# lpiccinelli-eth/UniDepth

Hardware: NVIDIA H100
Metric: images/sec UniDepthV2.infer ViT-L/14 480x640 (higher is better)
Workload: dtype f16 operands, f32 accumulate/residual

## Files before the change

include/udb.h:

```cpp
#ifndef UDB_H_
#define UDB_H_
#include <stddef.h>
#include <stdint.h>

#ifdef __cplusplus
extern "C" {
#endif

#define UDB_VERSION 1

int udb_version(void);

typedef struct udb_profile_entry_t {
  char name[48];
  float ms;
  double flops;
  double bytes;
} udb_profile_entry_t;
int udb_profile_begin(void* stream);
int udb_profile_end(udb_profile_entry_t* out, int32_t cap);
const char* udb_last_error(void);
int64_t udb_launch_count(void);

enum { UDB_A_MATRIX = 0, UDB_A_CONV3X3 = 1 };
enum { UDB_ACT_NONE = 0, UDB_ACT_GELU = 1, UDB_ACT_LEAKY = 2 };
enum { UDB_STORE_ROWS = 0, UDB_STORE_CONVT = 1, UDB_STORE_CONVTILE = 2, UDB_STORE_HEAD = 3 };

typedef struct udb_gemm_t {
  const void* a;
  const void* w;
  int32_t M, N, K;
  int32_t lda, ldw;
  int32_t a_mode;
  int32_t conv_B, conv_H, conv_W, conv_C, conv_inH, conv_inW, conv_off, conv_TH, conv_TW;
  int32_t conv_cstride, conv_coff;
  const float* bias;
  const float* gamma;
  const void* resid;
  int32_t resid_f32;
  void* out;
  int32_t out_f32;
  void* out2;
  int32_t out2_leaky;
  int32_t act;
  int32_t store_mode;
  int64_t ldc;
  int32_t rows_per_group, group_stride, row_offset;
  int32_t resid_mod, resid_row_offset;
  int64_t ldr;
  int32_t ct_k, ct_cout, ct_h, ct_w, ct_pad;
  const float* head_w;
  float head_b, head_add;
  int32_t a_split_k;
  int32_t out_split;
  float* ln_stats_out;
  const float* ln_stats_in;
  const float* ln_c1;
  int32_t ln_parts, ln_part_cols;
  float ln_eps;
} udb_gemm_t;

int udb_gemm_f16(const udb_gemm_t* g, void* stream);

typedef struct udb_conv_halo_t {
  const void* x;
  const void* w;
  const float* bias;
  int32_t B, H, W, C, cstride, coff, cout, act;
  void* out;
  int64_t ldc;
  const float* head_w;
  float head_b, head_add;
  float* head_out;
} udb_conv_halo_t;
int udb_conv3x3_halo_f16(const udb_conv_halo_t* c, void* stream);

typedef struct udb_attn_t {
  const void* q;
  const void* k;
  const void* v;
  void* out;
  int32_t B, heads, seq_q, seq_k, head_dim;
  int32_t ldq, ldk, ldv, ldo;
  int32_t q_col0, k_col0, v_col0, o_col0;
  float scale;
  int32_t split;
  int32_t lo_off_q, lo_off_k, lo_off_v, lo_off_o;
} udb_attn_t;

int udb_attention_f16(const udb_attn_t* a, void* stream);

typedef struct udb_layernorm_t {
  const void* in;
  int32_t in_f32;
  void* out;
  int32_t out_f32;
  const float* weight;
  const float* bias;
  int32_t rows, dim;
  int64_t ld_in, ld_out;
  int32_t rows_per_group, group_stride, row_offset;
  float eps;
  int32_t dim_valid;
  int32_t out_split;
} udb_layernorm_t;

int udb_layernorm(const udb_layernorm_t* p, void* stream);

typedef struct udb_preprocess_t {
  const void* rgb;
  int32_t rgb_is_u8;
  int32_t normalize;
  int32_t B, H, W;
  int32_t pad_l, pad_r, pad_t, pad_b;
  int32_t net_h, net_w;
  void* patches;
  int32_t ldp;
  int32_t split;
} udb_preprocess_t;

int udb_preprocess_patchify(const udb_preprocess_t* p, void* stream);

int udb_posembed_bicubic(const float* grid, int32_t m, int32_t dim, float* out, int32_t gh,
                         int32_t gw, void* stream);

int udb_set_cls_rows(float* x, const float* cls_token, const float* pos0, int32_t B, int32_t T,
                     int32_t D, void* stream);
int udb_set_cls_rows_ln(float* x, void* x16, float* stats, const float* cls_token, const float* pos0, int32_t B, int32_t T,
                        int32_t D, int32_t parts, int32_t part_cols, void* stream);

typedef struct udb_small_linear_t {
  const float* x;
  const float* w;
  const float* bias;
  const float* gamma;
  const float* resid;
  float* y;
  int32_t M, N, K;
  int32_t act;
  int32_t ldx, ldy, ldr;
} udb_small_linear_t;
int udb_small_linear_f32(const udb_small_linear_t* p, void* stream);

int udb_camera_attn4_f32(const float* q, const float* kv, const float* pos, float* out, int32_t B,
                         int32_t C, int32_t heads, void* stream);

int udb_camera_intrinsics(const float* x, int32_t B, int32_t net_h, int32_t net_w, float factor,
                          int32_t pad_l, int32_t pad_t, float* intr4, float* k_net, float* k_out,
                          void* stream);

int udb_camera_adjust_k(const float* K, int32_t B, float factor, int32_t pad_l, int32_t pad_t,
                        float* intr4, void* stream);

typedef struct udb_ray_embed_t {
  const float* intr4;
  const float* rays_in;
  const float* scales;
  int32_t B, net_h, net_w, gh, gw, bands;
  void* out;
  int32_t out_f32;
} udb_ray_embed_t;
int udb_ray_embed(const udb_ray_embed_t* p, void* stream);

int udb_upsample2x_nhwc_f16(const void* in, void* out, int32_t B, int32_t H, int32_t W, int32_t C,
                            void* stream);

int udb_resize_ac_pad_nhwc_f16(const void* in, void* out, int32_t B, int32_t H, int32_t W,
                               int32_t C, int32_t oh, int32_t ow, int32_t pad, void* stream);

int udb_reflect_pad1_nhwc_f16(const void* in, void* out, int32_t B, int32_t H, int32_t W, int32_t C,
                              void* stream);

int udb_reflect_border_fill_nhwc_f16(void* buf, int32_t B, int32_t H, int32_t W, int32_t C, void* stream);


typedef struct udb_v1_preprocess_t {
  const void* rgb;
  int32_t rgb_is_u8, scale255, normalize;
  int32_t B, H, W;
  int32_t rh, rw, pad_l, pad_t;
  int32_t net_h, net_w;
  int32_t patch;
  void* patches;
} udb_v1_preprocess_t;
int udb_v1_preprocess(const udb_v1_preprocess_t* p, void* stream);

int udb_vit_tap(const float* x, void* acc, float* cls_out, int32_t B, int32_t N, int32_t D, int32_t first, void* stream);

typedef struct udb_layernorm_any_t {
  const void* in;
  int32_t in_f32;
  void* out;
  int32_t out_f32;
  const float* weight;
  const float* bias;
  int64_t rows;
  int32_t dim;
  int64_t ld_in, ld_out;
  float eps;
  const float* add;
  int64_t add_mod;
  int32_t s2d_h, s2d_w;
} udb_layernorm_any_t;
int udb_layernorm_any(const udb_layernorm_any_t* p, void* stream);

int udb_dwconv7_nhwc_f16(const void* x, const float* w, const float* bias, void* y, int32_t B, int32_t H, int32_t W,
                         int32_t C, void* stream);

int udb_max_accum_f16(const void* src, void* dst, int64_t n, int32_t first, void* stream);

int udb_spatial_mean_f32(const float* x, float* out, int32_t B, int32_t HW, int32_t C, void* stream);

int udb_aa_resize_nhwc_f16(const void* in, void* out, int32_t B, int32_t H, int32_t W, int32_t C, int32_t oh, int32_t ow,
                           void* stream);

typedef struct udb_v1_rays_t {
  const float* intr4;
  int32_t B, net_h, net_w, gh, gw;
  const float* ln_w;
  const float* ln_b;
  void* out;
  float sh_k[81];
} udb_v1_rays_t;
int udb_v1_rays_sh81(const udb_v1_rays_t* p, void* stream);

int udb_v1_camera_intrinsics(const float* x4, const float* gt_k, int32_t B, int32_t net_h, int32_t net_w, float ratio,
                             int32_t pad_l, int32_t pad_t, int32_t skip_camera, float* intr4_rays, float* k_out,
                             float* k4_points, void* stream);

int udb_cross_attn_small(const float* q, const float* q_pos, const void* kv, float* out, float* scratch, int32_t B, int32_t nq,
                         int32_t nk, int32_t D, float scale, void* stream);

int udb_softmax_rows(const float* s, void* p, int64_t rows, int32_t n_valid, int32_t ld_in, int32_t ld_out, float scale,
                     void* stream);

int udb_add_f32(const float* a, const float* b, float* out, void* out_f16, int64_t n, void* stream);

int udb_copy_rows_f32_to_f16(const float* src, void* dst, int32_t groups, int32_t rows_per_group, int32_t D,
                             int64_t dst_group_stride, int64_t dst_row0, void* stream);

int udb_conv3x3_c1_exp(const void* x, const float* w, float bias, float* out, int32_t B, int32_t H, int32_t W, int32_t C,
                       void* stream);

int udb_nystrom_landmarks(const void* q, int32_t ldq, const void* kv, int32_t ldkv, void* out, int32_t B, int32_t n,
                          int32_t heads, void* stream);
int udb_nystrom_k2_pinv(const void* landmarks, float* k2, float* z, float* tmp, int32_t B, int32_t heads, int32_t iters,
                        void* stream);
int udb_nystrom_zk3(const float* z, const void* k3, int32_t ldk3, void* out, int32_t ldo, int32_t B, int32_t heads, void* stream);

int udb_v1_mean_maps(const float* o8, const float* o4, const float* o2, float* mean, int32_t B, int32_t gh, int32_t gw,
                     int32_t net_h, int32_t net_w, void* stream);
typedef struct udb_v1_postprocess_t {
  const float* mean;
  const float* k4;
  int32_t B, net_h, net_w, pad_l, pad_r, pad_t, pad_b, H, W;
  float* out_depth;
  float* out_points;
} udb_v1_postprocess_t;
int udb_v1_postprocess(const udb_v1_postprocess_t* p, void* stream);

typedef struct udb_postprocess_t {
  const float* radius;
  const float* confidence;
  const float* intr4;
  const float* rays_in;
  int32_t B, net_h, net_w, padded_h, padded_w, pad_l, pad_t, H, W;
  float* out_confidence;
  float* out_radius;
  float* out_depth;
  float* out_points;
  float* out_rays;
} udb_postprocess_t;
int udb_postprocess(const udb_postprocess_t* p, void* stream);

typedef struct udb_engine udb_engine;

enum { UDB_DT_F16 = 0, UDB_DT_F32 = 1 };

typedef struct udb_config_t {
  int32_t embed_dim, depth, enc_heads;
  int32_t taps[4];
  int32_t pos_grid;
  int32_t hidden, dec_heads, expansion, out_dim;
  int32_t n_stages;
  int32_t dec_depths[4];
  double ratio_min, ratio_max;
  double pixels_min, pixels_max;
} udb_config_t;

int udb_create(const udb_config_t* cfg, udb_engine** out);
void udb_destroy(udb_engine* e);

int udb_set_weight(udb_engine* e, const char* name, const void* dev_ptr, const int64_t* shape, int32_t ndim,
                   int32_t dtype);
int udb_set_scalar(udb_engine* e, const char* name, double value);

typedef struct udb_geometry_t {
  int32_t pad_l, pad_r, pad_t, pad_b;
  int32_t padded_h, padded_w;
  int32_t net_h, net_w;
  int32_t gh, gw;
  double factor;
} udb_geometry_t;
#define UDB_LEVEL_NETWORK_ONLY (-2)
int udb_geometry(const udb_engine* e, int32_t H, int32_t W, int32_t resolution_level, udb_geometry_t* out);

size_t udb_workspace_bytes(udb_engine* e, int32_t B, int32_t H, int32_t W, int32_t resolution_level);
size_t udb_schedule_bytes(udb_engine* e, int32_t B, int32_t H, int32_t W, int32_t resolution_level);

typedef struct udb_infer_args_t {
  const void* rgb;
  int32_t rgb_is_u8, normalize;
  int32_t B, H, W;
  int32_t resolution_level;
  const float* camera_k;
  const float* camera_rays;
  const float* ray_scales;
  void* workspace;
  size_t workspace_bytes;
  float* confidence;
  float* intrinsics;
  float* radius;
  float* depth;
  float* points;
  float* rays;
  float* depth_features;
} udb_infer_args_t;

int udb_infer_v2(udb_engine* e, const udb_infer_args_t* a, void* stream);

typedef struct udb_engine_v1 udb_engine_v1;

#define UDB_V1_ENCODER_CONVNEXT 0
#define UDB_V1_ENCODER_DINOV2 1

typedef struct udb_v1_config_t {
  int32_t depths[4];
  int32_t dims[4];
  int32_t hidden, heads, expansion;
  int32_t dec_depths[3];
  int32_t encoder;
  int32_t net_h, net_w;
} udb_v1_config_t;

int udb_v1_create(const udb_v1_config_t* cfg, udb_engine_v1** out);
void udb_v1_destroy(udb_engine_v1* e);
int udb_v1_set_weight(udb_engine_v1* e, const char* name, const void* dev_ptr, const int64_t* shape, int32_t ndim,
                      int32_t dtype);
int udb_v1_set_scalar(udb_engine_v1* e, const char* name, double value);
typedef struct udb_v1_geometry_t {
  int32_t resized_h, resized_w;
  int32_t pad_l, pad_r, pad_t, pad_b;
  double ratio;
} udb_v1_geometry_t;
int udb_v1_geometry(int32_t H, int32_t W, int32_t net_h, int32_t net_w, udb_v1_geometry_t* out);
size_t udb_v1_workspace_bytes(udb_engine_v1* e, int32_t B, int32_t H, int32_t W);

typedef struct udb_infer_v1_args_t {
  const void* rgb;
  int32_t rgb_is_u8;
  int32_t scale255;
  int32_t normalize;
  int32_t B, H, W;
  const float* intrinsics;
  int32_t skip_camera;
  void* workspace;
  size_t workspace_bytes;
  float* out_intrinsics;
  float* out_points;
  float* out_depth;
} udb_infer_v1_args_t;

int udb_infer_v1(udb_engine_v1* e, const udb_infer_v1_args_t* a, void* stream);

int udb_p2p_alloc(size_t bytes, void** dev_ptr, void* handle64);
int udb_p2p_open(const void* handle64, void** peer_ptr);
int udb_p2p_close(void* peer_ptr);
int udb_p2p_free(void* dev_ptr);
int udb_p2p_barrier(void* const* peer_flags_dev, void* my_flags, int32_t rank, int32_t world, uint32_t epoch,
                    int32_t* timeout_flag_dev, void* stream);
int udb_p2p_copy(void* dst, const void* src, size_t bytes, void* stream);

#ifdef __cplusplus
}
#endif
#endif
```

unidepth_b200/_cabi.py:

```python
from __future__ import annotations

import ctypes as C
import os

_HERE = os.path.dirname(os.path.abspath(__file__))
LIB_PATH = os.environ.get("UDB_LIB", os.path.join(_HERE, "libudb.so"))

A_MATRIX, A_CONV3X3 = 0, 1
ACT_NONE, ACT_GELU, ACT_LEAKY = 0, 1, 2
STORE_ROWS, STORE_CONVT, STORE_CONVTILE, STORE_HEAD = 0, 1, 2, 3

vp, i32, i64, f32 = C.c_void_p, C.c_int32, C.c_int64, C.c_float


class Gemm(C.Structure):
    _fields_ = [
        ("a", vp), ("w", vp), ("M", i32), ("N", i32), ("K", i32), ("lda", i32), ("ldw", i32),
        ("a_mode", i32),
        ("conv_B", i32), ("conv_H", i32), ("conv_W", i32), ("conv_C", i32), ("conv_inH", i32),
        ("conv_inW", i32), ("conv_off", i32), ("conv_TH", i32), ("conv_TW", i32),
        ("conv_cstride", i32), ("conv_coff", i32),
        ("bias", vp), ("gamma", vp), ("resid", vp), ("resid_f32", i32), ("out", vp), ("out_f32", i32),
        ("out2", vp), ("out2_leaky", i32), ("act", i32), ("store_mode", i32), ("ldc", i64),
        ("rows_per_group", i32), ("group_stride", i32), ("row_offset", i32),
        ("resid_mod", i32), ("resid_row_offset", i32), ("ldr", i64),
        ("ct_k", i32), ("ct_cout", i32), ("ct_h", i32), ("ct_w", i32), ("ct_pad", i32),
        ("head_w", vp), ("head_b", f32), ("head_add", f32),
        ("a_split_k", i32), ("out_split", i32),
        ("ln_stats_out", vp), ("ln_stats_in", vp), ("ln_c1", vp), ("ln_parts", i32), ("ln_part_cols", i32), ("ln_eps", f32),
    ]


class ConvHalo(C.Structure):
    _fields_ = [
        ("x", vp), ("w", vp), ("bias", vp),
        ("B", i32), ("H", i32), ("W", i32), ("C", i32), ("cstride", i32), ("coff", i32), ("cout", i32), ("act", i32),
        ("out", vp), ("ldc", i64), ("head_w", vp), ("head_b", f32), ("head_add", f32), ("head_out", vp),
    ]


class Attn(C.Structure):
    _fields_ = [
        ("q", vp), ("k", vp), ("v", vp), ("out", vp),
        ("B", i32), ("heads", i32), ("seq_q", i32), ("seq_k", i32), ("head_dim", i32),
        ("ldq", i32), ("ldk", i32), ("ldv", i32), ("ldo", i32),
        ("q_col0", i32), ("k_col0", i32), ("v_col0", i32), ("o_col0", i32), ("scale", f32),
        ("split", i32), ("lo_off_q", i32), ("lo_off_k", i32), ("lo_off_v", i32), ("lo_off_o", i32),
    ]


class LayerNorm(C.Structure):
    _fields_ = [
        ("inp", vp), ("in_f32", i32), ("out", vp), ("out_f32", i32), ("weight", vp), ("bias", vp),
        ("rows", i32), ("dim", i32), ("ld_in", i64), ("ld_out", i64),
        ("rows_per_group", i32), ("group_stride", i32), ("row_offset", i32), ("eps", f32), ("dim_valid", i32),
        ("out_split", i32),
    ]


class Preprocess(C.Structure):
    _fields_ = [
        ("rgb", vp), ("rgb_is_u8", i32), ("normalize", i32), ("B", i32), ("H", i32), ("W", i32),
        ("pad_l", i32), ("pad_r", i32), ("pad_t", i32), ("pad_b", i32), ("net_h", i32), ("net_w", i32),
        ("patches", vp), ("ldp", i32), ("split", i32),
    ]


class SmallLinear(C.Structure):
    _fields_ = [
        ("x", vp), ("w", vp), ("bias", vp), ("gamma", vp), ("resid", vp), ("y", vp),
        ("M", i32), ("N", i32), ("K", i32), ("act", i32), ("ldx", i32), ("ldy", i32), ("ldr", i32),
    ]


class RayEmbed(C.Structure):
    _fields_ = [
        ("intr4", vp), ("rays_in", vp), ("scales", vp),
        ("B", i32), ("net_h", i32), ("net_w", i32), ("gh", i32), ("gw", i32), ("bands", i32),
        ("out", vp), ("out_f32", i32),
    ]


class Postprocess(C.Structure):
    _fields_ = [
        ("radius", vp), ("confidence", vp), ("intr4", vp), ("rays_in", vp),
        ("B", i32), ("net_h", i32), ("net_w", i32), ("padded_h", i32), ("padded_w", i32),
        ("pad_l", i32), ("pad_t", i32), ("H", i32), ("W", i32),
        ("out_confidence", vp), ("out_radius", vp), ("out_depth", vp), ("out_points", vp), ("out_rays", vp),
    ]


class Config(C.Structure):
    _fields_ = [
        ("embed_dim", i32), ("depth", i32), ("enc_heads", i32), ("taps", i32 * 4), ("pos_grid", i32),
        ("hidden", i32), ("dec_heads", i32), ("expansion", i32), ("out_dim", i32), ("n_stages", i32),
        ("dec_depths", i32 * 4),
        ("ratio_min", C.c_double), ("ratio_max", C.c_double), ("pixels_min", C.c_double), ("pixels_max", C.c_double),
    ]


class Geometry(C.Structure):
    _fields_ = [
        ("pad_l", i32), ("pad_r", i32), ("pad_t", i32), ("pad_b", i32), ("padded_h", i32), ("padded_w", i32),
        ("net_h", i32), ("net_w", i32), ("gh", i32), ("gw", i32), ("factor", C.c_double),
    ]


class V1Geometry(C.Structure):
    _fields_ = [
        ("resized_h", i32), ("resized_w", i32), ("pad_l", i32), ("pad_r", i32), ("pad_t", i32), ("pad_b", i32),
        ("ratio", C.c_double),
    ]


class InferArgs(C.Structure):
    _fields_ = [
        ("rgb", vp), ("rgb_is_u8", i32), ("normalize", i32), ("B", i32), ("H", i32), ("W", i32),
        ("resolution_level", i32), ("camera_k", vp), ("camera_rays", vp), ("ray_scales", vp), ("workspace", vp),
        ("workspace_bytes", C.c_size_t),
        ("confidence", vp), ("intrinsics", vp), ("radius", vp), ("depth", vp), ("points", vp), ("rays", vp),
        ("depth_features", vp),
    ]


class V1Preprocess(C.Structure):
    _fields_ = [
        ("rgb", vp), ("rgb_is_u8", i32), ("scale255", i32), ("normalize", i32), ("B", i32), ("H", i32), ("W", i32),
        ("rh", i32), ("rw", i32), ("pad_l", i32), ("pad_t", i32), ("net_h", i32), ("net_w", i32), ("patch", i32),
        ("patches", vp),
    ]


class LayerNormAny(C.Structure):
    _fields_ = [
        ("inp", vp), ("in_f32", i32), ("out", vp), ("out_f32", i32), ("weight", vp), ("bias", vp),
        ("rows", i64), ("dim", i32), ("ld_in", i64), ("ld_out", i64), ("eps", f32), ("add", vp), ("add_mod", i64),
        ("s2d_h", i32), ("s2d_w", i32),
    ]


class V1Rays(C.Structure):
    _fields_ = [
        ("intr4", vp), ("B", i32), ("net_h", i32), ("net_w", i32), ("gh", i32), ("gw", i32),
        ("ln_w", vp), ("ln_b", vp), ("out", vp), ("sh_k", f32 * 81),
    ]


class V1Postprocess(C.Structure):
    _fields_ = [
        ("mean", vp), ("k4", vp), ("B", i32), ("net_h", i32), ("net_w", i32), ("pad_l", i32), ("pad_r", i32),
        ("pad_t", i32), ("pad_b", i32), ("H", i32), ("W", i32), ("out_depth", vp), ("out_points", vp),
    ]


class V1Config(C.Structure):
    _fields_ = [
        ("depths", i32 * 4), ("dims", i32 * 4), ("hidden", i32), ("heads", i32), ("expansion", i32),
        ("dec_depths", i32 * 3), ("encoder", i32), ("net_h", i32), ("net_w", i32),
    ]


class InferV1Args(C.Structure):
    _fields_ = [
        ("rgb", vp), ("rgb_is_u8", i32), ("scale255", i32), ("normalize", i32), ("B", i32), ("H", i32), ("W", i32),
        ("intrinsics", vp), ("skip_camera", i32), ("workspace", vp), ("workspace_bytes", C.c_size_t),
        ("out_intrinsics", vp), ("out_points", vp), ("out_depth", vp),
    ]


class ProfileEntry(C.Structure):
    _fields_ = [("name", C.c_char * 48), ("ms", f32), ("flops", C.c_double), ("bytes", C.c_double)]


DT_F16, DT_F32 = 0, 1

EXPORTS = {
    "udb_version": (i32, []),
    "udb_last_error": (C.c_char_p, []),
    "udb_launch_count": (i64, []),
    "udb_profile_begin": (i32, [vp]),
    "udb_profile_end": (i32, [C.POINTER(ProfileEntry), i32]),
    "udb_gemm_f16": (i32, [C.POINTER(Gemm), vp]),
    "udb_conv3x3_halo_f16": (i32, [C.POINTER(ConvHalo), vp]),
    "udb_attention_f16": (i32, [C.POINTER(Attn), vp]),
    "udb_layernorm": (i32, [C.POINTER(LayerNorm), vp]),
    "udb_preprocess_patchify": (i32, [C.POINTER(Preprocess), vp]),
    "udb_posembed_bicubic": (i32, [vp, i32, i32, vp, i32, i32, vp]),
    "udb_set_cls_rows": (i32, [vp, vp, vp, i32, i32, i32, vp]),
    "udb_set_cls_rows_ln": (i32, [vp, vp, vp, vp, vp, i32, i32, i32, i32, i32, vp]),
    "udb_small_linear_f32": (i32, [C.POINTER(SmallLinear), vp]),
    "udb_camera_attn4_f32": (i32, [vp, vp, vp, vp, i32, i32, i32, vp]),
    "udb_camera_intrinsics": (i32, [vp, i32, i32, i32, f32, i32, i32, vp, vp, vp, vp]),
    "udb_ray_embed": (i32, [C.POINTER(RayEmbed), vp]),
    "udb_upsample2x_nhwc_f16": (i32, [vp, vp, i32, i32, i32, i32, vp]),
    "udb_resize_ac_pad_nhwc_f16": (i32, [vp, vp, i32, i32, i32, i32, i32, i32, i32, vp]),
    "udb_reflect_pad1_nhwc_f16": (i32, [vp, vp, i32, i32, i32, i32, vp]),
    "udb_reflect_border_fill_nhwc_f16": (i32, [vp, i32, i32, i32, i32, vp]),
    "udb_postprocess": (i32, [C.POINTER(Postprocess), vp]),
    "udb_camera_adjust_k": (i32, [vp, i32, f32, i32, i32, vp, vp]),
    "udb_create": (i32, [C.POINTER(Config), C.POINTER(vp)]),
    "udb_destroy": (None, [vp]),
    "udb_set_weight": (i32, [vp, C.c_char_p, vp, C.POINTER(i64), i32, i32]),
    "udb_set_scalar": (i32, [vp, C.c_char_p, C.c_double]),
    "udb_geometry": (i32, [vp, i32, i32, i32, C.POINTER(Geometry)]),
    "udb_workspace_bytes": (C.c_size_t, [vp, i32, i32, i32, i32]),
    "udb_schedule_bytes": (C.c_size_t, [vp, i32, i32, i32, i32]),
    "udb_infer_v2": (i32, [vp, C.POINTER(InferArgs), vp]),
    "udb_v1_preprocess": (i32, [C.POINTER(V1Preprocess), vp]),
    "udb_layernorm_any": (i32, [C.POINTER(LayerNormAny), vp]),
    "udb_dwconv7_nhwc_f16": (i32, [vp, vp, vp, vp, i32, i32, i32, i32, vp]),
    "udb_max_accum_f16": (i32, [vp, vp, i64, i32, vp]),
    "udb_spatial_mean_f32": (i32, [vp, vp, i32, i32, i32, vp]),
    "udb_vit_tap": (i32, [vp, vp, vp, i32, i32, i32, i32, vp]),
    "udb_aa_resize_nhwc_f16": (i32, [vp, vp, i32, i32, i32, i32, i32, i32, vp]),
    "udb_v1_rays_sh81": (i32, [C.POINTER(V1Rays), vp]),
    "udb_v1_camera_intrinsics": (i32, [vp, vp, i32, i32, i32, f32, i32, i32, i32, vp, vp, vp, vp]),
    "udb_cross_attn_small": (i32, [vp, vp, vp, vp, vp, i32, i32, i32, i32, f32, vp]),
    "udb_softmax_rows": (i32, [vp, vp, i64, i32, i32, i32, f32, vp]),
    "udb_add_f32": (i32, [vp, vp, vp, vp, i64, vp]),
    "udb_copy_rows_f32_to_f16": (i32, [vp, vp, i32, i32, i32, i64, i64, vp]),
    "udb_conv3x3_c1_exp": (i32, [vp, vp, f32, vp, i32, i32, i32, i32, vp]),
    "udb_nystrom_landmarks": (i32, [vp, i32, vp, i32, vp, i32, i32, i32, vp]),
    "udb_nystrom_k2_pinv": (i32, [vp, vp, vp, vp, i32, i32, i32, vp]),
    "udb_nystrom_zk3": (i32, [vp, vp, i32, vp, i32, i32, i32, vp]),
    "udb_v1_mean_maps": (i32, [vp, vp, vp, vp, i32, i32, i32, i32, i32, vp]),
    "udb_v1_postprocess": (i32, [C.POINTER(V1Postprocess), vp]),
    "udb_v1_create": (i32, [C.POINTER(V1Config), C.POINTER(vp)]),
    "udb_v1_destroy": (None, [vp]),
    "udb_v1_set_weight": (i32, [vp, C.c_char_p, vp, C.POINTER(i64), i32, i32]),
    "udb_v1_set_scalar": (i32, [vp, C.c_char_p, C.c_double]),
    "udb_v1_geometry": (i32, [i32, i32, i32, i32, C.POINTER(V1Geometry)]),
    "udb_v1_workspace_bytes": (C.c_size_t, [vp, i32, i32, i32]),
    "udb_infer_v1": (i32, [vp, C.POINTER(InferV1Args), vp]),
    "udb_p2p_alloc": (i32, [C.c_size_t, C.POINTER(vp), vp]),
    "udb_p2p_open": (i32, [vp, C.POINTER(vp)]),
    "udb_p2p_close": (i32, [vp]),
    "udb_p2p_free": (i32, [vp]),
    "udb_p2p_barrier": (i32, [vp, vp, i32, i32, C.c_uint32, vp, vp]),
    "udb_p2p_copy": (i32, [vp, vp, C.c_size_t, vp]),
}

_lib = None


def lib():
    global _lib
    if _lib is None:
        if not os.path.exists(LIB_PATH):
            raise RuntimeError(
                f"{LIB_PATH} not found: build the CUDA extension first (python -m unidepth_b200.build). "
                "unidepth_b200 has no CPU / PyTorch fallback.")
        l = C.CDLL(LIB_PATH)
        for name, (res, args) in EXPORTS.items():
            if "UDB_LIB" in os.environ and not hasattr(l, name):
                continue
            fn = getattr(l, name)
            fn.restype = res
            fn.argtypes = args
        _lib = l
    return _lib


def check(rc: int, what: str):
    if rc != 0:
        raise RuntimeError(f"{what} failed: {lib().udb_last_error().decode()}")


def profile(fn, stream_ptr, cap: int = 4096):
    l = lib()
    check(l.udb_profile_begin(stream_ptr), "udb_profile_begin")
    try:
        fn()
    finally:
        buf = (ProfileEntry * cap)()
        n = l.udb_profile_end(buf, cap)
    if n < 0:
        raise RuntimeError(f"udb_profile_end failed: {l.udb_last_error().decode()}")
    return [(buf[i].name.decode(), buf[i].ms, buf[i].flops, buf[i].bytes) for i in range(min(n, cap))]


def launch_count() -> int:
    return int(lib().udb_launch_count())
```

unidepth_b200/csrc/engine.cu:

```cuda
#include "engine_common.h"

namespace udb {

struct ShapeTables {
  float* pos = nullptr;
  float* scales = nullptr;
};

constexpr int PATCH = 14;

}

struct udb_engine : udb::EngineBase {
  udb_config_t cfg;
  std::unordered_map<long long, udb::ShapeTables> tables;
  std::unordered_map<std::string, size_t> ws_need;
};

namespace udb {

static inline int floordiv2(int v) { return v >= 0 ? v / 2 : -((-v + 1) / 2); }

static void paddings(int H, int W, double lo, double hi, udb_geometry_t* g) {
  const double ratio = static_cast<double>(W) / H;
  const double target = fmin(hi, fmax(lo, ratio));
  g->pad_l = g->pad_r = g->pad_t = g->pad_b = 0;
  if (ratio > target) {
    const int h_new = static_cast<int>(W / target);
    g->pad_t = floordiv2(h_new - H);
    g->pad_b = h_new - H - g->pad_t;
    g->padded_h = h_new;
    g->padded_w = W;
  } else {
    const int w_new = static_cast<int>(H * target);
    g->pad_l = floordiv2(w_new - W);
    g->pad_r = w_new - W - g->pad_l;
    g->padded_h = H;
    g->padded_w = w_new;
  }
}

static int resize(const udb_config_t& c, int level, udb_geometry_t* g) {
  double lo = c.pixels_min, hi = c.pixels_max;
  if (level >= 0) {
    if (level >= 10) { set_error("resolution_level should be in [0, 10)"); return 1; }
    const double interval = (hi - lo) / 10;
    const double l2 = level * interval + lo, h2 = (level + 1) * interval + lo;
    lo = l2;
    hi = h2;
  }
  const double n_ori = static_cast<double>(g->padded_w) * g->padded_h;
  const double target = fmin(hi, fmax(lo, n_ori));
  g->factor = pow(target / n_ori, 0.5);
  const int new_w = static_cast<int>(g->padded_w * g->factor);
  const int new_h = static_cast<int>(g->padded_h * g->factor);
  g->net_h = static_cast<int>(ceil(static_cast<double>(new_h) / PATCH)) * PATCH;
  g->net_w = static_cast<int>(ceil(static_cast<double>(new_w) / PATCH)) * PATCH;
  g->gh = g->net_h / PATCH;
  g->gw = g->net_w / PATCH;
  return 0;
}

static int run(udb_engine* e, const udb_infer_args_t& a, const udb_geometry_t& g, const ShapeTables& tb, Arena& ar,
               void* st) {
  const udb_config_t& cf = e->cfg;
  Ctx c{e, &ar, st, ar.dry};
  const int B = a.B, nh = g.net_h, nw = g.net_w, gh = g.gh, gw = g.gw;
  const int N = gh * gw, T = N + 1, D = cf.embed_dim, hid = cf.hidden;
  const size_t BN = static_cast<size_t>(B) * N, BT = static_cast<size_t>(B) * T;

  Stage stage;
  stage.next("udb:preprocess+patch_embed");
  const bool sp = e->scalars.count("precision") && e->scalars["precision"] == 1.0;
  const int sx = sp ? 2 : 1;
  const bool fuse = !sp && e->scalars.count("fuse_ln") && e->scalars["fuse_ln"] == 1.0;
  const int ln_bn = D % 256 == 0 ? 256 : (D % 192 == 0 ? 192 : (D % 128 == 0 ? 128 : 64));
  const int ln_parts = D / ln_bn * 2, ln_pc = ln_bn / 2;
  __half* x16 = fuse ? ar.h(BT * D) : nullptr;
  float* stats = fuse ? ar.f(BT * ln_parts * 2) : nullptr;
  __half* patches = ar.h(BN * 640 * sx);
  if (!c.dry) {
    udb_preprocess_t p;
    memset(&p, 0, sizeof(p));
    p.rgb = a.rgb; p.rgb_is_u8 = a.rgb_is_u8; p.normalize = a.normalize; p.B = B; p.H = a.H; p.W = a.W;
    p.pad_l = g.pad_l; p.pad_r = g.pad_r; p.pad_t = g.pad_t; p.pad_b = g.pad_b; p.net_h = nh; p.net_w = nw;
    p.patches = patches; p.ldp = 640 * sx; p.split = sp ? 1 : 0;
    c.done(udb_preprocess_patchify(&p, st));
  }
  float* x = ar.f(BT * D);
  {
    Ctx::G q{patches, c.H("patch_w"), static_cast<int>(BN), D, sp ? 3 * 640 : 640};
    q.lda = 640 * sx; q.a_split_k = sp ? 640 : 0;
    q.bias = c.F("patch_b"); q.resid = tb.pos; q.resid_f32 = 1; q.ldr = D; q.out = x; q.out_f32 = 1;
    q.rows_per_group = N; q.group_stride = T; q.row_offset = 1; q.resid_mod = N; q.resid_row_offset = 1;
    c.expect2("patch_w", D, sp ? 3 * 640 : 640);
    if (fuse) { q.out2 = x16; q.out2_leaky = 0; q.ln_stats_out = stats; q.ln_parts = ln_parts; q.ln_part_cols = ln_pc; }
    c.gemm(q);
    if (!c.dry && !c.rc)
      c.done(fuse ? udb_set_cls_rows_ln(x, x16, stats, c.F("cls"), tb.pos, B, T, D, ln_parts, ln_pc, st)
                  : udb_set_cls_rows(x, c.F("cls"), tb.pos, B, T, D, st));
  }

  stage.next("udb:encoder_blocks");
  __half* feats[4];
  float* clss[4];
  for (int l = 0; l < 4; ++l) { feats[l] = ar.h(BN * D); clss[l] = ar.f(static_cast<size_t>(B) * D); }
  {
    VitBlocks v{B, T, D, cf.enc_heads, cf.depth};
    v.split = sp; v.fuse = fuse; v.x16 = x16; v.stats = stats; v.ln_parts = ln_parts; v.ln_pc = ln_pc;
    int tap = 0;
    vit_blocks(c, "blocks.", x, v, [&](int i) {
      if (tap < 4 && i + 1 == cf.taps[tap]) {
        c.layernorm(x, 1, feats[tap], 0, c.F("norm_w"), c.F("norm_b"), static_cast<int>(BN), D, 1e-5f, N, T, 1);
        c.layernorm(x, 1, clss[tap], 1, c.F("norm_w"), c.F("norm_b"), B, D, 1e-5f, 1, T, 0);
        ++tap;
      }
    });
    if (tap != 4 && !c.rc) { set_error("engine: taps must be 4 increasing block indices <= depth"); c.rc = 1; }
  }

  stage.next("udb:adapters+camera_head");
  float* Fl[4];
  for (int l = 0; l < 4; ++l) {
    Fl[l] = ar.f(BN * hid);
    Ctx::G q{feats[l], c.H(idx("adapt.%d.w", l)), static_cast<int>(BN), hid, D};
    q.bias = c.F(idx("adapt.%d.b", l)); q.out = Fl[l]; q.out_f32 = 1;
    c.gemm(q);
  }
  float* tokens = ar.f(static_cast<size_t>(B) * 4 * hid);
  for (int l = 0; l < 4; ++l)
    c.small_linear(clss[l], B, D, c.F(idx("cam_adapt.%d.w", l)), hid, c.F(idx("cam_adapt.%d.b", l)), UDB_ACT_NONE, nullptr,
                   nullptr, tokens + l * hid, D, 4 * hid, 0);

  const int R4 = B * 4;
  float* t = cam_mlp(c, "cam.project", tokens, R4, hid, hid, hid, nullptr, nullptr);
  for (int k = 1; k <= 2; ++k) {
    const std::string ag = idx("cam.agg%d", k);
    float* xn = ar.f(static_cast<size_t>(R4) * hid);
    float* cn = ar.f(static_cast<size_t>(R4) * hid);
    c.layernorm(t, 1, xn, 1, c.F(ag + ".nxw"), c.F(ag + ".nxb"), R4, hid, 1e-5f);
    c.layernorm(t, 1, cn, 1, c.F(ag + ".ncw"), c.F(ag + ".ncb"), R4, hid, 1e-5f);
    float* q = ar.f(static_cast<size_t>(R4) * hid);
    float* kv = ar.f(static_cast<size_t>(R4) * 2 * hid);
    c.small_linear(xn, R4, hid, c.F(ag + ".q"), hid, nullptr, UDB_ACT_NONE, nullptr, nullptr, q);
    c.small_linear(cn, R4, hid, c.F(ag + ".kv"), 2 * hid, nullptr, UDB_ACT_NONE, nullptr, nullptr, kv);
    float* a4 = ar.f(static_cast<size_t>(R4) * hid);
    if (!c.dry && !c.rc) c.done(udb_camera_attn4_f32(q, kv, c.F("cam.pos"), a4, B, hid, cf.dec_heads, st));
    float* t2 = ar.f(static_cast<size_t>(R4) * hid);
    c.small_linear(a4, R4, hid, c.F(ag + ".out"), hid, nullptr, UDB_ACT_NONE, c.F(ag + ".ls1"), t, t2);
    t = cam_mlp(c, ag + ".mlp", t2, R4, hid, cf.expansion * hid, hid, t2, c.F(ag + ".ls2"));
  }
  float* x4 = cam_mlp(c, "cam.pinhole", t, R4, hid, hid, 1, nullptr, nullptr);
  float* intr4 = ar.f(static_cast<size_t>(B) * 4);
  float* k_net = ar.f(static_cast<size_t>(B) * 9);
  if (!c.dry && !c.rc)
    c.done(udb_camera_intrinsics(x4, B, nh, nw, static_cast<float>(g.factor), g.pad_l, g.pad_t, intr4, k_net, a.intrinsics, st));

  stage.next("udb:ray_embedding+prompt_blocks");
  const float* ray_intr = intr4;
  if (a.camera_k && !a.camera_rays) {
    float* gt4 = ar.f(static_cast<size_t>(B) * 4);
    if (!c.dry && !c.rc) c.done(udb_camera_adjust_k(a.camera_k, B, static_cast<float>(g.factor), g.pad_l, g.pad_t, gt4, st));
    ray_intr = gt4;
  }
  float* remb = ar.f(BN * hid);
  if (!c.dry && !c.rc) {
    udb_ray_embed_t p;
    memset(&p, 0, sizeof(p));
    p.intr4 = ray_intr; p.rays_in = a.camera_rays; p.scales = a.ray_scales ? a.ray_scales : tb.scales;
    p.B = B; p.net_h = nh; p.net_w = nw; p.gh = gh; p.gw = gw; p.bands = hid / 2; p.out = remb; p.out_f32 = 1;
    c.done(udb_ray_embed(&p, st));
  }

  __half* cond[4];
  for (int l = 0; l < 4; ++l) cond[l] = ar.h(BN * hid);
  const int hd = hid / cf.dec_heads;
  const int hp = cf.dec_heads * 64;
  {
    const size_t m = ar.mark();
    __half* xn = ar.h(BN * hid);
    __half* cn = ar.h(BN * hid);
    __half* qb = ar.h(BN * hp);
    __half* kvb = ar.h(BN * 2 * hp);
    __half* ab = ar.h(BN * hp);
    __half* mb = ar.h(BN * cf.expansion * hid);
    const float scale = static_cast<float>(pow(static_cast<double>(hd), -0.5));
    for (int l = 0; l < 4; ++l) {
      const std::string p = idx("prompt.%d.", l);
      c.layernorm(Fl[l], 1, xn, 0, c.F(p + "nxw"), c.F(p + "nxb"), static_cast<int>(BN), hid, 1e-5f);
      c.layernorm(remb, 1, cn, 0, c.F(p + "ncw"), c.F(p + "ncb"), static_cast<int>(BN), hid, 1e-5f);
      { Ctx::G q{xn, c.H(p + "q"), static_cast<int>(BN), hp, hid}; q.out = qb; c.gemm(q); }
      { Ctx::G q{cn, c.H(p + "kv"), static_cast<int>(BN), 2 * hp, hid}; q.out = kvb; c.gemm(q); }
      c.attention(qb, kvb, kvb, ab, B, cf.dec_heads, N, N, hp, 2 * hp, 2 * hp, hp, 0, 0, hp, scale);
      { Ctx::G q{ab, c.H(p + "out"), static_cast<int>(BN), hid, hp}; q.resid = Fl[l]; q.resid_f32 = 1; q.out = Fl[l];
        q.out_f32 = 1; c.gemm(q); }
      c.layernorm(Fl[l], 1, xn, 0, c.F(p + "mnw"), c.F(p + "mnb"), static_cast<int>(BN), hid, 1e-5f);
      { Ctx::G q{xn, c.H(p + "w1"), static_cast<int>(BN), cf.expansion * hid, hid}; q.bias = c.F(p + "b1");
        q.act = UDB_ACT_GELU; q.out = mb; c.gemm(q); }
      { Ctx::G q{mb, c.H(p + "w2"), static_cast<int>(BN), hid, cf.expansion * hid}; q.bias = c.F(p + "b2");
        q.resid = Fl[l]; q.resid_f32 = 1; q.out = cond[l]; c.gemm(q); }
    }
    ar.release(m);
  }

  stage.next("udb:upsampling_stages");
  { Ctx::G q{cond[0], c.H("lat_w"), static_cast<int>(BN), hid, hid}; q.bias = c.F("lat_b"); q.out = a.depth_features;
    q.out_f32 = 1; c.gemm(q); }
  const void* prev = a.depth_features;
  int prev_f32 = 1;
  int cur_h = gh, cur_w = gw, c_hr = 0;
  for (int i = 0; i < cf.n_stages; ++i) {
    const std::string s = idx("ups.%d.", i);
    const int k = i == 0 ? 1 : 2 * i;
    const Weight* ctw = c.W(s + "ct_w");
    const int cout = static_cast<int>(ctw->shape[0]) / (k * k);
    const int oh = cur_h, ow = cur_w;
    const size_t px = static_cast<size_t>(B) * oh * ow;
    __half* nxt = nullptr;
    const int up_c = static_cast<int>(c.W(s + "up_w")->shape[0]);
    nxt = ar.h(px * 4 * up_c);
    const size_t m = ar.mark();
    float* lat = ar.f(px * cout);
    __half* act = ar.h(px * cout);
    __half* tmp = ar.h(px * cout);
    c.conv_transpose(cond[i + 1], static_cast<int>(BN), hid, ctw->p, k, cout, gh, gw, c.F(s + "ct_b"), prev, prev_f32, lat, 1,
                     act, 1, 0);
    for (int j = 0; j < cf.dec_depths[i]; ++j) {
      const std::string r = idx2("ups.%d.rcu.%d.", i, j);
      c.expect2(r + "w1", cout, 9 * cout);
      c.expect2(r + "w2", cout, 9 * cout);
      c.conv3x3(act, B, oh, ow, cout, c.H(r + "w1"), cout, c.F(r + "b1"), UDB_ACT_LEAKY, nullptr, nullptr, 0, tmp, 0,
                nullptr, 1);
      c.conv3x3(tmp, B, oh, ow, cout, c.H(r + "w2"), cout, c.F(r + "b2"), UDB_ACT_NONE, c.F(r + "gamma"), lat, 1, lat, 1,
                act, j + 1 < cf.dec_depths[i] ? 1 : 0);
    }
    __half* u = ar.h(px * up_c);
    { Ctx::G q{act, c.H(s + "up_w"), static_cast<int>(px), up_c, cout}; q.bias = c.F(s + "up_b"); q.out = u; c.gemm(q); }
    if (!c.dry && !c.rc) c.done(udb_upsample2x_nhwc_f16(u, nxt, B, oh, ow, up_c, st));
    ar.release(m);
    prev = nxt;
    prev_f32 = 0;
    cur_h = 2 * oh;
    cur_w = 2 * ow;
    c_hr = up_c;
  }
  const int hh = cur_h, hw = cur_w;
  const size_t hpx = static_cast<size_t>(B) * hh * hw;

  stage.next("udb:depth+confidence_heads");
  __half* xhat = ar.h(hpx * c_hr);
  const int nxt_last = (2 * hid) >> cf.n_stages;
  const int c_valid = nxt_last > cf.out_dim ? nxt_last : cf.out_dim;
  c.layernorm(prev, 0, xhat, 0, c.F("ln_ones"), c.F("ln_zeros"), static_cast<int>(hpx), c_hr, 1e-5f, 0, 0, 0,
              c_valid != c_hr ? c_valid : 0);
  const int n_mlp = static_cast<int>(c.W("head_mlp_w")->shape[0]);
  __half* mp = ar.h(static_cast<size_t>(B) * (hh + 2) * (hw + 2) * n_mlp);
  c.conv_transpose(xhat, static_cast<int>(hpx), c_hr, c.H("head_mlp_w"), 1, n_mlp, hh, hw, c.F("head_mlp_b"), nullptr, 0, mp,
                   0, nullptr, 1, 1);
  if (!c.dry && !c.rc) c.done(udb_reflect_border_fill_nhwc_f16(mp, B, hh, hw, n_mlp, st));
  float* planes[2];
  for (int i = 0; i < 2; ++i) {
    const std::string hn = idx("heads.%d.", i);
    const int lr_c = static_cast<int>(c.W(hn + "lr_w")->shape[0]);
    planes[i] = ar.f(static_cast<size_t>(B) * nh * nw);
    const size_t m = ar.mark();
    __half* lr = ar.h(hpx * lr_c);
    c.conv_halo(mp, B, hh, hw, n_mlp / 2, n_mlp, i * (n_mlp / 2), c.H(hn + "lr_w"), lr_c, c.F(hn + "lr_b"), UDB_ACT_NONE, lr,
                nullptr, 0.f, 0.f, nullptr);
    __half* up = ar.h(static_cast<size_t>(B) * (nh + 2) * (nw + 2) * lr_c);
    if (!c.dry && !c.rc) c.done(udb_resize_ac_pad_nhwc_f16(lr, up, B, hh, hw, lr_c, nh, nw, 1, st));
    c.conv_halo(up, B, nh, nw, lr_c, lr_c, 0, c.H(hn + "hr_w"), 32, c.F(hn + "hr_b"), UDB_ACT_LEAKY, nullptr,
                c.F(hn + "head_w"), static_cast<float>(c.S(hn + "head_b")), static_cast<float>(c.S(hn + "add")), planes[i]);
    ar.release(m);
  }

  stage.next("udb:postprocess");
  if (!c.dry && !c.rc) {
    udb_postprocess_t p;
    memset(&p, 0, sizeof(p));
    p.radius = planes[0]; p.confidence = planes[1]; p.intr4 = ray_intr; p.rays_in = a.camera_rays;
    p.B = B; p.net_h = nh; p.net_w = nw; p.padded_h = g.padded_h; p.padded_w = g.padded_w; p.pad_l = g.pad_l; p.pad_t = g.pad_t;
    p.H = a.H; p.W = a.W;
    p.out_confidence = a.confidence; p.out_radius = a.radius; p.out_depth = a.depth; p.out_points = a.points; p.out_rays = a.rays;
    c.done(udb_postprocess(&p, st));
  }
  if (!c.rc && ar.overflow) { set_error("engine: workspace too small (%zu bytes needed)", ar.peak); return 1; }
  return c.rc;
}

static void ray_scale_table(int gh, int gw, int bands, std::vector<float>& out) {
  const int mx = (gh > gw ? gh : gw) / 2;
  const float end = static_cast<float>(log2(static_cast<double>(mx)));
  const float step = bands > 1 ? end / static_cast<float>(bands - 1) : 0.f;
  out.resize(bands);
  for (int i = 0; i < bands; ++i) {
    const float v = i < bands / 2 ? step * i : end - step * (bands - 1 - i);
    out[i] = powf(2.0f, v);
  }
}

static const ShapeTables* prepare(udb_engine* e, const udb_geometry_t& g) {
  const long long key = (static_cast<long long>(g.gh) << 32) | static_cast<unsigned>(g.gw);
  auto it = e->tables.find(key);
  if (it != e->tables.end()) return &it->second;
  auto pw = e->w.find("pos");
  if (pw == e->w.end()) { set_error("engine: 'pos' must be registered before udb_workspace_bytes"); return nullptr; }
  const int D = e->cfg.embed_dim, m = e->cfg.pos_grid, N = g.gh * g.gw;
  ShapeTables tb;
  auto fail = [&tb](const char* why) -> const ShapeTables* {
    if (why) set_error("%s", why);
    cudaFree(tb.pos);
    cudaFree(tb.scales);
    return nullptr;
  };
  if (cudaMalloc(&tb.pos, static_cast<size_t>(N + 1) * D * 4) != cudaSuccess ||
      cudaMalloc(&tb.scales, static_cast<size_t>(e->cfg.hidden / 2) * 4) != cudaSuccess)
    return fail("engine: cudaMalloc of the per-shape tables failed");
  const float* pos = static_cast<const float*>(pw->second.p);
  cudaMemcpy(tb.pos, pos, static_cast<size_t>(D) * 4, cudaMemcpyDeviceToDevice);
  if (g.gh == m && g.gw == m) {
    cudaMemcpy(tb.pos + D, pos + D, static_cast<size_t>(N) * D * 4, cudaMemcpyDeviceToDevice);
  } else if (udb_posembed_bicubic(pos + D, m, D, tb.pos + D, g.gh, g.gw, nullptr)) {
    return fail(nullptr);
  }
  std::vector<float> sc;
  ray_scale_table(g.gh, g.gw, e->cfg.hidden / 2, sc);
  cudaMemcpy(tb.scales, sc.data(), sc.size() * 4, cudaMemcpyHostToDevice);
  if (cudaDeviceSynchronize() != cudaSuccess) return fail("engine: preparing the per-shape tables failed");
  return &(e->tables[key] = tb);
}

}

using namespace udb;

extern "C" {

int udb_create(const udb_config_t* cfg, udb_engine** out) {
  if (!cfg || !out) { set_error("udb_create: null argument"); return 1; }
  if (cfg->embed_dim <= 0 || cfg->embed_dim % 64 || cfg->embed_dim / cfg->enc_heads != 64) {
    set_error("udb_create: encoder needs 64-wide heads (embed_dim %d, heads %d)", cfg->embed_dim, cfg->enc_heads);
    return 1;
  }
  const int hd = cfg->dec_heads > 0 ? cfg->hidden / cfg->dec_heads : 0;
  if (hd <= 0 || hd > 64) { set_error("udb_create: decoder head dim %d not supported", hd); return 1; }
  if (cfg->n_stages < 1 || cfg->n_stages > 4) { set_error("udb_create: n_stages %d out of range", cfg->n_stages); return 1; }
  udb_engine* e = new udb_engine();
  e->cfg = *cfg;
  *out = e;
  return 0;
}

void udb_destroy(udb_engine* e) {
  if (!e) return;
  for (auto& kv : e->tables) {
    cudaFree(kv.second.pos);
    cudaFree(kv.second.scales);
  }
  delete e;
}

int udb_set_weight(udb_engine* e, const char* name, const void* dev_ptr, const int64_t* shape, int32_t ndim, int32_t dtype) {
  if (!e || !name || !dev_ptr || ndim < 0 || ndim > 4) { set_error("udb_set_weight: bad argument"); return 1; }
  if (reinterpret_cast<uintptr_t>(dev_ptr) & 15) { set_error("udb_set_weight(%s): pointer must be 16-byte aligned", name); return 1; }
  Weight w;
  w.p = dev_ptr;
  w.dtype = dtype;
  w.ndim = ndim;
  for (int i = 0; i < ndim; ++i) w.shape[i] = shape[i];
  e->w[name] = w;
  return 0;
}

int udb_set_scalar(udb_engine* e, const char* name, double value) {
  if (!e || !name) { set_error("udb_set_scalar: bad argument"); return 1; }
  e->scalars[name] = value;
  return 0;
}

int udb_geometry(const udb_engine* e, int32_t H, int32_t W, int32_t level, udb_geometry_t* out) {
  if (!e || !out || H <= 0 || W <= 0) { set_error("udb_geometry: bad argument"); return 1; }
  if (level == UDB_LEVEL_NETWORK_ONLY) {
    if (H % PATCH || W % PATCH) { set_error("network-only input %dx%d must be a multiple of %d", H, W, PATCH); return 1; }
    memset(out, 0, sizeof(*out));
    out->padded_h = out->net_h = H;
    out->padded_w = out->net_w = W;
    out->gh = H / PATCH;
    out->gw = W / PATCH;
    out->factor = 1.0;
    return 0;
  }
  paddings(H, W, e->cfg.ratio_min, e->cfg.ratio_max, out);
  return resize(e->cfg, level, out);
}

size_t udb_schedule_bytes(udb_engine* e, int32_t B, int32_t H, int32_t W, int32_t level) {
  if (!e || B <= 0) { set_error("udb_schedule_bytes: bad argument"); return 0; }
  udb_geometry_t g;
  if (udb_geometry(e, H, W, level, &g)) return 0;
  udb_infer_args_t a;
  memset(&a, 0, sizeof(a));
  a.B = B; a.H = H; a.W = W; a.resolution_level = level;
  a.camera_k = reinterpret_cast<const float*>(16);
  const ShapeTables none;
  Arena ar(nullptr, 0);
  if (run(e, a, g, none, ar, nullptr)) return 0;
  return ar.peak + 256;
}

size_t udb_workspace_bytes(udb_engine* e, int32_t B, int32_t H, int32_t W, int32_t level) {
  udb_geometry_t g;
  if (udb_geometry(e, H, W, level, &g)) return 0;
  const ShapeTables* tb = prepare(e, g);
  if (!tb) return 0;
  udb_infer_args_t a;
  memset(&a, 0, sizeof(a));
  a.B = B; a.H = H; a.W = W; a.resolution_level = level;
  a.camera_k = reinterpret_cast<const float*>(16);
  Arena ar(nullptr, 0);
  if (run(e, a, g, *tb, ar, nullptr)) return 0;
  char key[96];
  snprintf(key, sizeof(key), "%d,%d,%d,%d", B, H, W, level);
  e->ws_need[key] = ar.peak + 256;
  return ar.peak + 256;
}

int udb_infer_v2(udb_engine* e, const udb_infer_args_t* a, void* stream) {
  if (!e || !a || !a->rgb || !a->workspace) { set_error("udb_infer_v2: null argument"); return 1; }
  if (!a->confidence || !a->intrinsics || !a->radius || !a->depth || !a->points || !a->rays || !a->depth_features) {
    set_error("udb_infer_v2: all seven output pointers are required");
    return 1;
  }
  udb_geometry_t g;
  if (udb_geometry(e, a->H, a->W, a->resolution_level, &g)) return 1;
  const long long key = (static_cast<long long>(g.gh) << 32) | static_cast<unsigned>(g.gw);
  auto it = e->tables.find(key);
  char wkey[96];
  snprintf(wkey, sizeof(wkey), "%d,%d,%d,%d", a->B, a->H, a->W, a->resolution_level);
  auto need = e->ws_need.find(wkey);
  if (it == e->tables.end() || need == e->ws_need.end()) {
    set_error("udb_infer_v2: shape %dx%dx%d (level %d) not prepared; call udb_workspace_bytes first", a->B, a->H, a->W,
              a->resolution_level);
    return 1;
  }
  if (a->workspace_bytes < need->second) {
    set_error("udb_infer_v2: workspace too small (%zu bytes given, %zu needed)", a->workspace_bytes, need->second);
    return 1;
  }
  Arena ar(a->workspace, a->workspace_bytes);
  if (reinterpret_cast<uintptr_t>(a->workspace) & 255) { set_error("udb_infer_v2: workspace must be 256-byte aligned"); return 1; }
  return run(e, *a, g, it->second, ar, stream);
}

}
```

unidepth_b200/csrc/gemm.cu:

```cuda
#include "common.h"
#include "ptx.cuh"

namespace udb {

constexpr int BM = 128;
constexpr int BK = 64;
constexpr int kEpiWarps = 8;
constexpr int kTP = 36;
constexpr int kThreads = (kEpiWarps + 4) * 32;

struct GemmArgs {
  int M, N, K, num_kb;
  int tiles_m, tiles_n;
  int a_mode;
  int conv_B, conv_H, conv_W, conv_cpb , conv_off, conv_TH, conv_TW, conv_tx, conv_ty;
  const float* bias;
  const float* gamma;
  const void* resid;
  int resid_f32;
  void* out;
  int out_f32;
  __half* out2;
  int out2_leaky;
  int act;
  int store_mode;
  long long ldc, ldr;
  int rpg, gstride, roff;
  int resid_mod, resid_roff;
  int ct_k, ct_cout, ct_h, ct_w, ct_pad;
  int conv_coff;
  const float* head_w;
  float head_b, head_add;
  int a_wrap;
  int out_split;
  float* stats_out;
  const float* ln_stats;
  const float* ln_c1;
  int ln_parts, ln_part_cols;
  float ln_eps;
};

template <int BN>
struct GemmCfg {
  static constexpr int kStages = BN >= 256 ? 3 : (BN >= 192 ? 4 : (BN >= 128 ? 5 : 7));
  static constexpr int kABytes = BM * BK * 2;
  static constexpr int kBBytes = BN * BK * 2;
  static constexpr int kStageBytes = kABytes + kBBytes;
  static constexpr int kStagingBytes = kEpiWarps * (32 * kTP * 4 + 2 * 32 * 4);
  static constexpr int kSmemBytes = kStages * kStageBytes + kStagingBytes + 256 ;
  static_assert(kSmemBytes <= 232448, "shared memory per block");
};

struct EpiWarp {
  float* T;
  float* Twg;
  uint32_t* roff_out;
  uint32_t* roff_res;
  int wg, wq, grp, lane, r_in_tile;
};

template <int BN, bool LNF>
__device__ __forceinline__ void epilogue_tile(const GemmArgs& p, const EpiWarp& w, const float (&acc)[BN / 2], const int mt,
                                              const int nt) {
  constexpr int kGroups = BN >= 64 ? 2 : 1;
  constexpr int kColsPerGrp = BN / kGroups;
  const int grp = w.grp, lane = w.lane, r_in_tile = w.r_in_tile;
  const bool active = grp < kGroups;
  float* T = w.T;
  uint32_t* roff_out = w.roff_out;
  uint32_t* roff_res = w.roff_res;
  bool valid = false;
  long long out_off = 0, res_off = 0;
  uint32_t vmask = 0;
  float ln_mean = 0.f, ln_rstd = 1.f;
  float st_pivot = 0.f, st_s1 = 0.f, st_s2 = 0.f;
  bool st_first = true;
  if (active) {

    const int m = mt * BM + r_in_tile;
    if (p.store_mode == UDB_STORE_CONVTILE || p.store_mode == UDB_STORE_HEAD) {
      const int per_img = p.conv_tx * p.conv_ty;
      const int b = mt / per_img;
      const int r = mt % per_img;
      const int y = (r / p.conv_tx) * p.conv_TH + r_in_tile / p.conv_TW;
      const int x = (r % p.conv_tx) * p.conv_TW + r_in_tile % p.conv_TW;
      valid = (b < p.conv_B) && (y < p.conv_H) && (x < p.conv_W);
      out_off = (((long long)b * p.conv_H + y) * p.conv_W + x) * p.ldc;
      res_off = (((long long)b * p.conv_H + y) * p.conv_W + x) * p.ldr;
    } else if (p.store_mode == UDB_STORE_CONVT) {
      valid = m < p.M;
      const int hw = p.ct_h * p.ct_w;
      const int b = m / hw;
      const int r = m % hw;
      const int y = r / p.ct_w, x = r % p.ct_w;
      const long long W2 = (long long)p.ct_w * p.ct_k + 2 * p.ct_pad;
      const long long H2 = (long long)p.ct_h * p.ct_k + 2 * p.ct_pad;
      out_off = ((b * H2 + (long long)y * p.ct_k + p.ct_pad) * W2 + (long long)x * p.ct_k + p.ct_pad) * p.ct_cout;
      res_off = out_off;
    } else {
      valid = m < p.M;
      long long orow = m;
      if (p.rpg > 0) orow = (long long)(m / p.rpg) * p.gstride + (m % p.rpg) + p.roff;
      out_off = orow * p.ldc;
      res_off = (p.resid_mod > 0) ? ((long long)(m % p.resid_mod) + p.resid_roff) * p.ldr
                                  : orow * p.ldr;
    }
    vmask = __ballot_sync(0xffffffffu, valid);
    roff_out[lane] = static_cast<uint32_t>(out_off);
    roff_res[lane] = static_cast<uint32_t>(res_off);
    __syncwarp();
    if (LNF && p.ln_stats) {
      const float2* sp = reinterpret_cast<const float2*>(p.ln_stats) + (long long)(valid ? m : 0) * p.ln_parts;
      float ms = 0.f, m2 = 0.f;
      for (int q = 0; q < p.ln_parts; ++q) ms += sp[q].x;
      ln_mean = ms / (float)p.ln_parts;
      for (int q = 0; q < p.ln_parts; ++q) {
        const float2 t = sp[q];
        m2 += t.y + (float)p.ln_part_cols * (t.x - ln_mean) * (t.x - ln_mean);
      }
      ln_rstd = rsqrtf(m2 / (float)(p.ln_parts * p.ln_part_cols) + p.ln_eps);
    }
  }
  const int frow = 16 * (w.wq & 1) + (lane >> 2), fcol = 2 * (lane & 3);
#pragma unroll
  for (int c = 0; c < kColsPerGrp; c += 32) {
    bar_sync(1 + w.wg, 128);
#pragma unroll
    for (int gi = 0; gi < kGroups; ++gi) {
      float* Tt = w.Twg + ((w.wq >> 1) | (gi << 1)) * 32 * kTP;
#pragma unroll
      for (int j = 0; j < 4; ++j) {
        const int f = ((gi * kColsPerGrp + c) / 8 + j) * 4;
        *reinterpret_cast<float2*>(Tt + frow * kTP + 8 * j + fcol) = make_float2(acc[f], acc[f + 1]);
        *reinterpret_cast<float2*>(Tt + (frow + 8) * kTP + 8 * j + fcol) = make_float2(acc[f + 2], acc[f + 3]);
      }
    }
    bar_sync(1 + w.wg, 128);
    if (!active) continue;
    const int col = grp * kColsPerGrp + c;
    const int n0 = nt * BN + col;
    float v[32];
#pragma unroll
    for (int j = 0; j < 32; j += 4) {
      const float4 t = *reinterpret_cast<const float4*>(T + lane * kTP + j);
      v[j] = t.x; v[j + 1] = t.y; v[j + 2] = t.z; v[j + 3] = t.w;
    }
    __syncwarp();
    if (n0 >= p.N) continue;
    if (LNF && p.ln_stats) {
      const float4* cp = reinterpret_cast<const float4*>(p.ln_c1 + n0);
      const float mr = ln_mean * ln_rstd;
#pragma unroll
      for (int j = 0; j < 8; ++j) {
        const float4 c4 = __ldg(cp + j);
        v[4 * j] = fmaf(v[4 * j], ln_rstd, -mr * c4.x);
        v[4 * j + 1] = fmaf(v[4 * j + 1], ln_rstd, -mr * c4.y);
        v[4 * j + 2] = fmaf(v[4 * j + 2], ln_rstd, -mr * c4.z);
        v[4 * j + 3] = fmaf(v[4 * j + 3], ln_rstd, -mr * c4.w);
      }
    }
    if (p.bias) {
      const float4* bp = reinterpret_cast<const float4*>(p.bias + n0);
#pragma unroll
      for (int j = 0; j < 8; ++j) {
        const float4 b4 = __ldg(bp + j);
        v[4 * j] += b4.x; v[4 * j + 1] += b4.y; v[4 * j + 2] += b4.z; v[4 * j + 3] += b4.w;
      }
    }
    if (p.act == UDB_ACT_GELU) {
#pragma unroll
      for (int j = 0; j < 32; j += 2) gelu_erf_pair(v[j], v[j + 1]);
    } else if (p.act == UDB_ACT_LEAKY) {
#pragma unroll
      for (int j = 0; j < 32; ++j) v[j] = leaky(v[j]);
    }
    if (p.store_mode == UDB_STORE_HEAD) {
      float head = p.head_b;
#pragma unroll
      for (int j = 0; j < 32; ++j) head = fmaf(v[j], __ldg(p.head_w + j), head);
      head = fminf(fmaxf(head, -8.0f), 8.0f) + p.head_add;
      if (valid) reinterpret_cast<float*>(p.out)[out_off] = expf(head);
      continue;
    }
    if (p.gamma) {
      const float4* gp = reinterpret_cast<const float4*>(p.gamma + n0);
#pragma unroll
      for (int j = 0; j < 8; ++j) {
        const float4 g4 = __ldg(gp + j);
        v[4 * j] *= g4.x; v[4 * j + 1] *= g4.y; v[4 * j + 2] *= g4.z; v[4 * j + 3] *= g4.w;
      }
    }
    long long coff = n0;
    if (p.store_mode == UDB_STORE_CONVT) {
      const int tap = n0 / p.ct_cout;
      const int co = n0 % p.ct_cout;
      const long long W2 = (long long)p.ct_w * p.ct_k + 2 * p.ct_pad;
      coff = ((long long)(tap / p.ct_k) * W2 + (tap % p.ct_k)) * p.ct_cout + co;
    }
    const uint32_t c32 = static_cast<uint32_t>(coff);
    const int l4 = (lane & 7) * 4, rq = lane >> 3;
    float* Trow = T + lane * kTP;
    auto stage_rows = [&](const float (&x)[32]) {
#pragma unroll
      for (int j = 0; j < 32; j += 4)
        *reinterpret_cast<float4*>(Trow + j) = make_float4(x[j], x[j + 1], x[j + 2], x[j + 3]);
    };
    auto for_rows = [&](auto&& body) {
      if (vmask == 0xffffffffu) {
#pragma unroll
        for (int i = 0; i < 8; ++i) body(4 * i + rq, true);
      } else {
#pragma unroll
        for (int i = 0; i < 8; ++i) body(4 * i + rq, ((vmask >> (4 * i + rq)) & 1u) != 0);
      }
    };
    if (p.resid) {
      if (p.resid_f32) {
        const float* rp = reinterpret_cast<const float*>(p.resid) + c32 + l4;
        float4 tmp[8];
        int k = 0;
        for_rows([&](int rr, bool ok) {
          tmp[k++] = ok ? *reinterpret_cast<const float4*>(rp + roff_res[rr]) : make_float4(0.f, 0.f, 0.f, 0.f);
        });
#pragma unroll
        for (int i = 0; i < 8; ++i) *reinterpret_cast<float4*>(T + (4 * i + rq) * kTP + l4) = tmp[i];
      } else {
        const __half* rp = reinterpret_cast<const __half*>(p.resid) + c32 + l4;
        uint2 tmp[8];
        int k = 0;
        for_rows([&](int rr, bool ok) {
          tmp[k++] = ok ? *reinterpret_cast<const uint2*>(rp + roff_res[rr]) : make_uint2(0u, 0u);
        });
#pragma unroll
        for (int i = 0; i < 8; ++i) {
          const float2 a = __half22float2(*reinterpret_cast<const __half2*>(&tmp[i].x));
          const float2 b = __half22float2(*reinterpret_cast<const __half2*>(&tmp[i].y));
          *reinterpret_cast<float4*>(T + (4 * i + rq) * kTP + l4) = make_float4(a.x, a.y, b.x, b.y);
        }
      }
      __syncwarp();
#pragma unroll
      for (int j = 0; j < 32; j += 4) {
        const float4 t = *reinterpret_cast<const float4*>(Trow + j);
        v[j] += t.x; v[j + 1] += t.y; v[j + 2] += t.z; v[j + 3] += t.w;
      }
      __syncwarp();
    }
    if (LNF && p.stats_out) {
      if (st_first) { st_pivot = v[0]; st_first = false; }
#pragma unroll
      for (int j = 0; j < 32; ++j) {
        const float dlt = v[j] - st_pivot;
        st_s1 += dlt;
        st_s2 = fmaf(dlt, dlt, st_s2);
      }
    }
    if (p.out) {
      stage_rows(v);
      __syncwarp();
      if (p.out_f32) {
        float* op = reinterpret_cast<float*>(p.out) + c32 + l4;
        for_rows([&](int rr, bool ok) {
          if (ok) *reinterpret_cast<float4*>(op + roff_out[rr]) = *reinterpret_cast<const float4*>(T + rr * kTP + l4);
        });
      } else {
        __half* op = reinterpret_cast<__half*>(p.out) + c32 + l4;
        if (p.out_split == 0) {
          for_rows([&](int rr, bool ok) {
            const float4 t = *reinterpret_cast<const float4*>(T + rr * kTP + l4);
            if (ok) *reinterpret_cast<uint2*>(op + roff_out[rr]) = make_uint2(pack_half2(t.x, t.y), pack_half2(t.z, t.w));
          });
        } else {
          for_rows([&](int rr, bool ok) {
            const float4 t = *reinterpret_cast<const float4*>(T + rr * kTP + l4);
            const uint2 hi = make_uint2(pack_half2(t.x, t.y), pack_half2(t.z, t.w));
            const float2 h01 = __half22float2(*reinterpret_cast<const __half2*>(&hi.x));
            const float2 h23 = __half22float2(*reinterpret_cast<const __half2*>(&hi.y));
            if (ok) {
              *reinterpret_cast<uint2*>(op + roff_out[rr]) = hi;
              *reinterpret_cast<uint2*>(op + roff_out[rr] + p.out_split) =
                  make_uint2(pack_half2(t.x - h01.x, t.y - h01.y), pack_half2(t.z - h23.x, t.w - h23.y));
            }
          });
        }
      }
      __syncwarp();
    }
    if (p.out2) {
      if (p.out2_leaky) {
#pragma unroll
        for (int j = 0; j < 32; ++j) v[j] = leaky(v[j]);
        stage_rows(v);
      } else if (!p.out) {
        stage_rows(v);
      }
      __syncwarp();
      __half* op = p.out2 + c32 + l4;
      for_rows([&](int rr, bool ok) {
        const float4 t = *reinterpret_cast<const float4*>(T + rr * kTP + l4);
        if (ok) *reinterpret_cast<uint2*>(op + roff_out[rr]) = make_uint2(pack_half2(t.x, t.y), pack_half2(t.z, t.w));
      });
      __syncwarp();
    }
  }
  if (LNF && p.stats_out && active && valid && !st_first) {
    const float n = (float)kColsPerGrp;
    const float mean_p = st_pivot + st_s1 / n;
    const float m2_p = fmaxf(st_s2 - st_s1 * st_s1 / n, 0.f);
    const long long orow = out_off / p.ldc;
    reinterpret_cast<float2*>(p.stats_out)[orow * (p.tiles_n * kGroups) + nt * kGroups + grp] = make_float2(mean_p, m2_p);
  }
}

template <int BN, bool LNF>
__global__ void __launch_bounds__(kThreads, 1)
gemm_f16_kernel(const __grid_constant__ CUtensorMap tmA, const __grid_constant__ CUtensorMap tmB,
                const GemmArgs p) {
  using Cfg = GemmCfg<BN>;
  constexpr int kStages = Cfg::kStages;
  extern __shared__ __align__(1024) uint8_t smem[];
  uint8_t* sA = smem;
  uint8_t* sB = smem + kStages * Cfg::kABytes;
  uint8_t* staging = smem + kStages * Cfg::kStageBytes;
  uint64_t* bars = reinterpret_cast<uint64_t*>(staging + Cfg::kStagingBytes);
  uint64_t* full_bar = bars;
  uint64_t* empty_bar = bars + kStages;

  const int warp = threadIdx.x >> 5;
  const int lane = threadIdx.x & 31;
  pdl_launch_dependents();

  if (threadIdx.x == 0) {
    if (smem_u32(smem) & 1023) __trap();
    prefetch_tmap(&tmA);
    prefetch_tmap(&tmB);
    for (int i = 0; i < kStages; ++i) {
      mbar_init(&full_bar[i], 1);
      mbar_init(&empty_bar[i], kEpiWarps);
    }
    fence_barrier_init();
  }
  __syncthreads();
  pdl_wait();

  const int num_tiles = p.tiles_m * p.tiles_n;

  if (warp >= kEpiWarps) {
    setmaxnreg_dec<40>();
    if (warp != kEpiWarps) return;
    const bool elected = elect_one();
    int stage = 0;
    uint32_t phase = 0;
    for (int tile = blockIdx.x; tile < num_tiles; tile += gridDim.x) {
      const int mt = tile / p.tiles_n;
      const int nt = tile % p.tiles_n;
      int cb = 0, cy = 0, cx = 0;
      if (p.a_mode == UDB_A_CONV3X3) {
        const int per_img = p.conv_tx * p.conv_ty;
        cb = mt / per_img;
        const int r = mt % per_img;
        cy = (r / p.conv_tx) * p.conv_TH + p.conv_off;
        cx = (r % p.conv_tx) * p.conv_TW + p.conv_off;
      }
      for (int kb = 0; kb < p.num_kb; ++kb) {
        mbar_wait(&empty_bar[stage], phase ^ 1);
        if (elected) {
          mbar_arrive_expect_tx(&full_bar[stage], Cfg::kStageBytes);
          if (p.a_mode == UDB_A_CONV3X3) {
            const int tap = kb / p.conv_cpb;
            const int c0 = p.conv_coff + (kb % p.conv_cpb) * BK;
            tma_load_4d(sA + stage * Cfg::kABytes, &tmA, &full_bar[stage], c0, cx + tap % 3, cy + tap / 3, cb);
          } else {
            int ka = kb * BK;
            if (p.a_wrap && ka >= p.a_wrap) ka -= p.a_wrap;
            tma_load_2d(sA + stage * Cfg::kABytes, &tmA, &full_bar[stage], ka, mt * BM);
          }
          tma_load_2d(sB + stage * Cfg::kBBytes, &tmB, &full_bar[stage], kb * BK, nt * BN);
        }
        __syncwarp();
        if (++stage == kStages) {
          stage = 0;
          phase ^= 1;
        }
      }
    }
  } else {
    setmaxnreg_inc<232>();
    const int wg = warp >> 2, wq = warp & 3;
    float* Twg = reinterpret_cast<float*>(staging) + wg * 4 * 32 * kTP;
    uint32_t* roff = reinterpret_cast<uint32_t*>(staging + kEpiWarps * 32 * kTP * 4) + warp * 64;
    const EpiWarp ctx{Twg + wq * 32 * kTP, Twg, roff, roff + 32, wg, wq, wq >> 1, lane, 64 * wg + 32 * (wq & 1) + lane};
    float acc[BN / 2];
#pragma unroll
    for (int i = 0; i < BN / 2; ++i) acc[i] = 0.f;
    int stage = 0;
    uint32_t phase = 0;
    for (int tile = blockIdx.x; tile < num_tiles; tile += gridDim.x) {
      const int mt = tile / p.tiles_n;
      const int nt = tile % p.tiles_n;
      int prev = -1;
      for (int kb = 0; kb < p.num_kb; ++kb) {
        mbar_wait(&full_bar[stage], phase);
        const uint64_t da = gmma_desc_sw128(smem_u32(sA + stage * Cfg::kABytes + wg * 64 * 128), 16, 1024);
        const uint64_t db = gmma_desc_sw128(smem_u32(sB + stage * Cfg::kBBytes), 16, 1024);
        wgmma_fence();
#pragma unroll
        for (int k = 0; k < BK / 16; ++k) WgmmaSS<BN>::run(acc, da + 2 * k, db + 2 * k, (kb | k) != 0 ? 1u : 0u);
        wgmma_commit();
        wgmma_wait<1>();
        if (prev >= 0 && lane == 0) mbar_arrive(&empty_bar[prev]);
        prev = stage;
        if (++stage == kStages) {
          stage = 0;
          phase ^= 1;
        }
      }
      wgmma_wait<0>();
      wgmma_fence_regs(acc);
      if (prev >= 0 && lane == 0) mbar_arrive(&empty_bar[prev]);
      epilogue_tile<BN, LNF>(p, ctx, acc, mt, nt);
    }
  }
}

template <int BN, bool LNF>
static int launch_gemm(const CUtensorMap& tmA, const CUtensorMap& tmB, const GemmArgs& a, cudaStream_t st) {
  using Cfg = GemmCfg<BN>;
  static std::atomic<uint64_t> attr_mask{0};
  if (first_on_device(attr_mask)) {
    cudaError_t e = cudaFuncSetAttribute(gemm_f16_kernel<BN, LNF>, cudaFuncAttributeMaxDynamicSharedMemorySize,
                                         Cfg::kSmemBytes);
    if (e != cudaSuccess) {
      set_error("gemm: cudaFuncSetAttribute(%d B smem): %s", Cfg::kSmemBytes, cudaGetErrorString(e));
      return 1;
    }
  }
  const int tiles = a.tiles_m * a.tiles_n;
  const int grid = tiles < num_sms() ? tiles : num_sms();
  cudaError_t e = launch_ex(gemm_f16_kernel<BN, LNF>, dim3(grid), dim3(kThreads), Cfg::kSmemBytes, st, 1, tmA, tmB, a);
  if (e != cudaSuccess) {
    set_error("gemm_f16_kernel launch: %s", cudaGetErrorString(e));
    return 1;
  }
  return check_launch("gemm_f16_kernel");
}

}

extern "C" int udb_gemm_f16(const udb_gemm_t* g, void* stream) {
  using namespace udb;
  if (!g || !g->a || !g->w) { set_error("udb_gemm_f16: null operand"); return 1; }
  if (g->N % 32 != 0) { set_error("udb_gemm_f16: N=%d must be a multiple of 32", g->N); return 1; }
  GemmArgs a{};
  a.M = g->M; a.N = g->N; a.K = g->K;
  a.num_kb = (g->K + BK - 1) / BK;
  a.a_mode = g->a_mode;
  a.bias = g->bias; a.gamma = g->gamma; a.resid = g->resid; a.resid_f32 = g->resid_f32;
  a.out = g->out; a.out_f32 = g->out_f32; a.out2 = reinterpret_cast<__half*>(g->out2); a.out2_leaky = g->out2_leaky;
  a.act = g->act; a.store_mode = g->store_mode;
  a.ldc = g->ldc; a.ldr = g->ldr > 0 ? g->ldr : g->ldc;
  a.rpg = g->rows_per_group; a.gstride = g->group_stride; a.roff = g->row_offset;
  a.resid_mod = g->resid_mod; a.resid_roff = g->resid_row_offset;
  a.ct_k = g->ct_k; a.ct_cout = g->ct_cout; a.ct_h = g->ct_h; a.ct_w = g->ct_w; a.ct_pad = g->ct_pad;
  a.conv_coff = g->conv_coff;
  a.head_w = g->head_w; a.head_b = g->head_b; a.head_add = g->head_add;
  a.a_wrap = 0;
  a.out_split = g->out_split;
  if (g->a_split_k > 0) {
    if (g->a_mode != UDB_A_MATRIX || g->a_split_k % BK || g->K != 3 * g->a_split_k || g->lda < 2 * g->a_split_k) {
      set_error("udb_gemm_f16: split operands need a_mode MATRIX, K1 %% 64 == 0, K == 3*K1, lda >= 2*K1 (K1=%d K=%d lda=%d)",
                g->a_split_k, g->K, g->lda);
      return 1;
    }
    a.a_wrap = 2 * g->a_split_k;
  }
  a.stats_out = g->ln_stats_out; a.ln_stats = g->ln_stats_in; a.ln_c1 = g->ln_c1; a.ln_eps = g->ln_eps;
  a.ln_parts = g->ln_parts; a.ln_part_cols = g->ln_part_cols;
  if ((g->ln_stats_out || g->ln_stats_in) && g->store_mode != UDB_STORE_ROWS) {
    set_error("udb_gemm_f16: fused LayerNorm statistics need the ROWS store"); return 1;
  }
  if (g->ln_stats_in && (!g->ln_c1 || g->ln_parts <= 0 || g->ln_part_cols <= 0 || g->rows_per_group > 0)) {
    set_error("udb_gemm_f16: ln_stats_in needs ln_c1, ln_parts, ln_part_cols and an identity row map"); return 1;
  }
  if (g->out_split && (g->out_f32 || !g->out || g->store_mode != UDB_STORE_ROWS)) {
    set_error("udb_gemm_f16: out_split needs an f16 `out` with the ROWS store"); return 1;
  }

  int bn;
  if (g->store_mode == UDB_STORE_HEAD) {
    if (g->N != 32) { set_error("udb_gemm_f16: HEAD store needs N == 32"); return 1; }
    bn = 32;
  } else if (g->N % 256 == 0) bn = 256;
  else if (g->N % 192 == 0) bn = 192;
  else if (g->N % 128 == 0) bn = 128;
  else if (g->N % 64 == 0) bn = 64;
  else bn = 32;
  if (g->store_mode == UDB_STORE_CONVT && (g->ct_cout % 32) != 0) {
    set_error("udb_gemm_f16: CONVT needs Cout %% 32 == 0"); return 1;
  }
  a.tiles_n = (g->N + bn - 1) / bn;
  if (g->ln_stats_out) {
    const int groups = bn >= 64 ? 2 : 1;
    if (g->N % bn || g->ln_parts != a.tiles_n * groups || g->ln_part_cols != bn / groups) {
      set_error("udb_gemm_f16: ln_stats_out with N=%d runs as %d parts of %d columns (caller said %d x %d)", g->N, a.tiles_n * groups,
                bn / groups, g->ln_parts, g->ln_part_cols);
      return 1;
    }
  }

  CUtensorMap tmA, tmB;
  if (g->a_mode == UDB_A_CONV3X3) {
    if (g->conv_C % BK != 0 || g->K != 9 * g->conv_C) {
      set_error("udb_gemm_f16: conv3x3 needs C %% 64 == 0 and K == 9*C (C=%d K=%d)", g->conv_C, g->K);
      return 1;
    }
    if (g->store_mode != UDB_STORE_CONVTILE && g->store_mode != UDB_STORE_HEAD) {
      set_error("udb_gemm_f16: conv3x3 operand needs a CONVTILE or HEAD store"); return 1;
    }
    const int TH = g->conv_TH > 0 ? g->conv_TH : 8, TW = g->conv_TW > 0 ? g->conv_TW : 16;
    if (TH * TW != BM) { set_error("udb_gemm_f16: conv tile %dx%d != 128 pixels", TH, TW); return 1; }
    a.conv_B = g->conv_B; a.conv_H = g->conv_H; a.conv_W = g->conv_W; a.conv_cpb = g->conv_C / BK; a.conv_off = g->conv_off;
    a.conv_TH = TH; a.conv_TW = TW;
    a.conv_tx = (g->conv_W + TW - 1) / TW; a.conv_ty = (g->conv_H + TH - 1) / TH;
    a.tiles_m = g->conv_B * a.conv_tx * a.conv_ty;
    a.M = a.tiles_m * BM;
    const uint64_t cs = g->conv_cstride > 0 ? g->conv_cstride : g->conv_C;
    if ((uint64_t)g->conv_coff + g->conv_C > cs || (g->conv_coff % 8)) {
      set_error("udb_gemm_f16: bad conv channel slice (off %d, C %d, stride %d)", g->conv_coff, g->conv_C, (int)cs);
      return 1;
    }
    const uint64_t dims[4] = {cs, (uint64_t)g->conv_inW, (uint64_t)g->conv_inH, (uint64_t)g->conv_B};
    const uint64_t str[3] = {cs * 2, (uint64_t)g->conv_inW * cs * 2, (uint64_t)g->conv_inH * g->conv_inW * cs * 2};
    const uint32_t box[4] = {(uint32_t)BK, (uint32_t)TW, (uint32_t)TH, 1};
    if (make_tmap_f16(&tmA, g->a, 4, dims, str, box, true)) return 1;
  } else {
    a.tiles_m = (g->M + BM - 1) / BM;
    if (g->store_mode == UDB_STORE_CONVTILE || g->store_mode == UDB_STORE_HEAD) {
      set_error("udb_gemm_f16: tile store modes need a_mode == CONV3X3"); return 1;
    }
    const uint64_t dims[2] = {(uint64_t)(g->a_split_k > 0 ? 2 * g->a_split_k : g->K), (uint64_t)g->M};
    const uint64_t str[1] = {(uint64_t)g->lda * 2};
    const uint32_t box[2] = {(uint32_t)BK, (uint32_t)BM};
    if (make_tmap_f16(&tmA, g->a, 2, dims, str, box, true)) return 1;
  }
  {
    const uint64_t dims[2] = {(uint64_t)g->K, (uint64_t)g->N};
    const uint64_t str[1] = {(uint64_t)g->ldw * 2};
    const uint32_t box[2] = {(uint32_t)BK, (uint32_t)bn};
    if (make_tmap_f16(&tmB, g->w, 2, dims, str, box, true)) return 1;
  }
  cudaStream_t st = reinterpret_cast<cudaStream_t>(stream);
  note_work(2.0 * a.M * (double)g->N * g->K,
            2.0 * ((double)a.M * (g->a_mode == UDB_A_CONV3X3 ? g->conv_C : (g->a_split_k ? 2 * g->a_split_k : g->K)) + (double)g->N * g->K) +
                (double)a.M * g->N * ((g->out ? (g->out_f32 ? 4 : 2) : 0) + (g->out2 ? 2 : 0) + (g->resid ? (g->resid_f32 ? 4 : 2) : 0)));
  const bool lnf = g->ln_stats_out || g->ln_stats_in;
  if (lnf) {
    switch (bn) {
      case 256: return launch_gemm<256, true>(tmA, tmB, a, st);
      case 192: return launch_gemm<192, true>(tmA, tmB, a, st);
      case 128: return launch_gemm<128, true>(tmA, tmB, a, st);
      case 64: return launch_gemm<64, true>(tmA, tmB, a, st);
      default: return launch_gemm<32, true>(tmA, tmB, a, st);
    }
  }
  switch (bn) {
    case 256: return launch_gemm<256, false>(tmA, tmB, a, st);
    case 192: return launch_gemm<192, false>(tmA, tmB, a, st);
    case 128: return launch_gemm<128, false>(tmA, tmB, a, st);
    case 64: return launch_gemm<64, false>(tmA, tmB, a, st);
    default: return launch_gemm<32, false>(tmA, tmB, a, st);
  }
}
```

unidepth_b200/csrc/ptx.cuh:

```cuda
#pragma once
#include <cuda_fp16.h>
#include <cuda_runtime.h>
#include <stdint.h>
#include <stdio.h>

namespace udb {

__device__ __forceinline__ uint32_t smem_u32(const void* p) {
  return static_cast<uint32_t>(__cvta_generic_to_shared(p));
}

__device__ __forceinline__ bool elect_one() {
  uint32_t pred = 0;
  asm volatile(
      "{\n\t"
      ".reg .b32 rx;\n\t"
      ".reg .pred px;\n\t"
      "elect.sync rx|px, 0xffffffff;\n\t"
      "selp.b32 %0, 1, 0, px;\n\t"
      "}\n"
      : "=r"(pred));
  return pred != 0;
}

__device__ __forceinline__ void pdl_launch_dependents() {
  asm volatile("griddepcontrol.launch_dependents;" ::: "memory");
}
__device__ __forceinline__ void pdl_wait() { asm volatile("griddepcontrol.wait;" ::: "memory"); }

__device__ __forceinline__ void mbar_init(uint64_t* bar, uint32_t count) {
  asm volatile("mbarrier.init.shared::cta.b64 [%0], %1;" ::"r"(smem_u32(bar)), "r"(count));
}
__device__ __forceinline__ void fence_barrier_init() {
  asm volatile("fence.mbarrier_init.release.cluster;" ::: "memory");
}
__device__ __forceinline__ void mbar_arrive(uint64_t* bar) {
  asm volatile("mbarrier.arrive.shared::cta.b64 _, [%0];" ::"r"(smem_u32(bar)) : "memory");
}
__device__ __forceinline__ void mbar_arrive_expect_tx(uint64_t* bar, uint32_t bytes) {
  asm volatile("mbarrier.arrive.expect_tx.shared::cta.b64 _, [%0], %1;" ::"r"(smem_u32(bar)),
               "r"(bytes)
               : "memory");
}
__device__ __forceinline__ bool mbar_try_wait(uint64_t* bar, uint32_t parity) {
  uint32_t ok;
  asm volatile(
      "{\n\t"
      ".reg .pred p;\n\t"
      "mbarrier.try_wait.parity.shared::cta.b64 p, [%1], %2, %3;\n\t"
      "selp.b32 %0, 1, 0, p;\n\t"
      "}\n"
      : "=r"(ok)
      : "r"(smem_u32(bar)), "r"(parity), "r"(20000u)
      : "memory");
  return ok != 0;
}
#ifndef UDB_SPIN_LIMIT
#define UDB_SPIN_LIMIT (1u << 22)
#endif
__device__ __forceinline__ void mbar_wait(uint64_t* bar, uint32_t parity) {
  if (mbar_try_wait(bar, parity)) return;
  uint32_t spins = 0;
  while (!mbar_try_wait(bar, parity)) {
    if (++spins > UDB_SPIN_LIMIT) __trap();
  }
}

__device__ __forceinline__ void fence_proxy_async_smem() {
  asm volatile("fence.proxy.async.shared::cta;" ::: "memory");
}

__device__ __forceinline__ void prefetch_tmap(const void* tmap) {
  asm volatile("prefetch.tensormap [%0];" ::"l"(reinterpret_cast<uint64_t>(tmap)) : "memory");
}
__device__ __forceinline__ void tma_load_2d(void* smem_dst, const void* tmap, uint64_t* bar, int c0,
                                            int c1) {
  asm volatile(
      "cp.async.bulk.tensor.2d.shared::cluster.global.mbarrier::complete_tx::bytes"
      " [%0], [%1, {%3, %4}], [%2];" ::"r"(smem_u32(smem_dst)),
      "l"(reinterpret_cast<uint64_t>(tmap)), "r"(smem_u32(bar)), "r"(c0), "r"(c1)
      : "memory");
}
__device__ __forceinline__ void tma_load_3d(void* smem_dst, const void* tmap, uint64_t* bar, int c0,
                                            int c1, int c2) {
  asm volatile(
      "cp.async.bulk.tensor.3d.shared::cluster.global.mbarrier::complete_tx::bytes"
      " [%0], [%1, {%3, %4, %5}], [%2];" ::"r"(smem_u32(smem_dst)),
      "l"(reinterpret_cast<uint64_t>(tmap)), "r"(smem_u32(bar)), "r"(c0), "r"(c1), "r"(c2)
      : "memory");
}
__device__ __forceinline__ void tma_load_4d(void* smem_dst, const void* tmap, uint64_t* bar, int c0,
                                            int c1, int c2, int c3) {
  asm volatile(
      "cp.async.bulk.tensor.4d.shared::cluster.global.mbarrier::complete_tx::bytes"
      " [%0], [%1, {%3, %4, %5, %6}], [%2];" ::"r"(smem_u32(smem_dst)),
      "l"(reinterpret_cast<uint64_t>(tmap)), "r"(smem_u32(bar)), "r"(c0), "r"(c1), "r"(c2), "r"(c3)
      : "memory");
}


__device__ __forceinline__ void wgmma_fence() { asm volatile("wgmma.fence.sync.aligned;" ::: "memory"); }
__device__ __forceinline__ void wgmma_commit() { asm volatile("wgmma.commit_group.sync.aligned;" ::: "memory"); }
template <int N>
__device__ __forceinline__ void wgmma_wait() {
  asm volatile("wgmma.wait_group.sync.aligned %0;" ::"n"(N) : "memory");
}
template <int R>
__device__ __forceinline__ void wgmma_fence_regs(float (&d)[R]) {
#pragma unroll
  for (int i = 0; i < R; ++i) asm volatile("" : "+f"(d[i])::"memory");
}
template <uint32_t R>
__device__ __forceinline__ void setmaxnreg_inc() { asm volatile("setmaxnreg.inc.sync.aligned.u32 %0;" ::"n"(R)); }
template <uint32_t R>
__device__ __forceinline__ void setmaxnreg_dec() { asm volatile("setmaxnreg.dec.sync.aligned.u32 %0;" ::"n"(R)); }
__device__ __forceinline__ void bar_sync(int id, int threads) {
  asm volatile("bar.sync %0, %1;" ::"r"(id), "r"(threads) : "memory");
}

__device__ __forceinline__ uint64_t gmma_desc_sw128(uint32_t smem_addr, uint32_t lbo_bytes, uint32_t sbo_bytes) {
  uint64_t d = 0;
  d |= static_cast<uint64_t>((smem_addr & 0x3FFFF) >> 4);
  d |= static_cast<uint64_t>((lbo_bytes >> 4) & 0x3FFF) << 16;
  d |= static_cast<uint64_t>((sbo_bytes >> 4) & 0x3FFF) << 32;
  d |= static_cast<uint64_t>(1) << 62;
  return d;
}

__device__ __forceinline__ void wgmma_ss_n32(float (&d)[16], uint64_t da, uint64_t db, uint32_t scale_d) {
  asm volatile(
      "{\n\t.reg .pred p;\n\tsetp.ne.b32 p, %18, 0;\n\t"
      "wgmma.mma_async.sync.aligned.m64n32k16.f32.f16.f16 {%0, %1, %2, %3, %4, %5, %6, %7, %8, %9, %10, %11, %12, %13, %14, %15}, %16, %17, p, 1, 1, 0, 0;\n\t}\n"
      : "+f"(d[0]), "+f"(d[1]), "+f"(d[2]), "+f"(d[3]), "+f"(d[4]), "+f"(d[5]), "+f"(d[6]), "+f"(d[7]), "+f"(d[8]), "+f"(d[9]), "+f"(d[10]), "+f"(d[11]), "+f"(d[12]), "+f"(d[13]), "+f"(d[14]), "+f"(d[15])
      : "l"(da), "l"(db), "r"(scale_d));
}
__device__ __forceinline__ void wgmma_ss_n64(float (&d)[32], uint64_t da, uint64_t db, uint32_t scale_d) {
  asm volatile(
      "{\n\t.reg .pred p;\n\tsetp.ne.b32 p, %34, 0;\n\t"
      "wgmma.mma_async.sync.aligned.m64n64k16.f32.f16.f16 {%0, %1, %2, %3, %4, %5, %6, %7, %8, %9, %10, %11, %12, %13, %14, %15, %16, %17, %18, %19, %20, %21, %22, %23, %24, %25, %26, %27, %28, %29, %30, %31}, %32, %33, p, 1, 1, 0, 0;\n\t}\n"
      : "+f"(d[0]), "+f"(d[1]), "+f"(d[2]), "+f"(d[3]), "+f"(d[4]), "+f"(d[5]), "+f"(d[6]), "+f"(d[7]), "+f"(d[8]), "+f"(d[9]), "+f"(d[10]), "+f"(d[11]), "+f"(d[12]), "+f"(d[13]), "+f"(d[14]), "+f"(d[15]), "+f"(d[16]), "+f"(d[17]), "+f"(d[18]), "+f"(d[19]), "+f"(d[20]), "+f"(d[21]), "+f"(d[22]), "+f"(d[23]), "+f"(d[24]), "+f"(d[25]), "+f"(d[26]), "+f"(d[27]), "+f"(d[28]), "+f"(d[29]), "+f"(d[30]), "+f"(d[31])
      : "l"(da), "l"(db), "r"(scale_d));
}
__device__ __forceinline__ void wgmma_ss_n128(float (&d)[64], uint64_t da, uint64_t db, uint32_t scale_d) {
  asm volatile(
      "{\n\t.reg .pred p;\n\tsetp.ne.b32 p, %66, 0;\n\t"
      "wgmma.mma_async.sync.aligned.m64n128k16.f32.f16.f16 {%0, %1, %2, %3, %4, %5, %6, %7, %8, %9, %10, %11, %12, %13, %14, %15, %16, %17, %18, %19, %20, %21, %22, %23, %24, %25, %26, %27, %28, %29, %30, %31, %32, %33, %34, %35, %36, %37, %38, %39, %40, %41, %42, %43, %44, %45, %46, %47, %48, %49, %50, %51, %52, %53, %54, %55, %56, %57, %58, %59, %60, %61, %62, %63}, %64, %65, p, 1, 1, 0, 0;\n\t}\n"
      : "+f"(d[0]), "+f"(d[1]), "+f"(d[2]), "+f"(d[3]), "+f"(d[4]), "+f"(d[5]), "+f"(d[6]), "+f"(d[7]), "+f"(d[8]), "+f"(d[9]), "+f"(d[10]), "+f"(d[11]), "+f"(d[12]), "+f"(d[13]), "+f"(d[14]), "+f"(d[15]), "+f"(d[16]), "+f"(d[17]), "+f"(d[18]), "+f"(d[19]), "+f"(d[20]), "+f"(d[21]), "+f"(d[22]), "+f"(d[23]), "+f"(d[24]), "+f"(d[25]), "+f"(d[26]), "+f"(d[27]), "+f"(d[28]), "+f"(d[29]), "+f"(d[30]), "+f"(d[31]), "+f"(d[32]), "+f"(d[33]), "+f"(d[34]), "+f"(d[35]), "+f"(d[36]), "+f"(d[37]), "+f"(d[38]), "+f"(d[39]), "+f"(d[40]), "+f"(d[41]), "+f"(d[42]), "+f"(d[43]), "+f"(d[44]), "+f"(d[45]), "+f"(d[46]), "+f"(d[47]), "+f"(d[48]), "+f"(d[49]), "+f"(d[50]), "+f"(d[51]), "+f"(d[52]), "+f"(d[53]), "+f"(d[54]), "+f"(d[55]), "+f"(d[56]), "+f"(d[57]), "+f"(d[58]), "+f"(d[59]), "+f"(d[60]), "+f"(d[61]), "+f"(d[62]), "+f"(d[63])
      : "l"(da), "l"(db), "r"(scale_d));
}
__device__ __forceinline__ void wgmma_ss_n192(float (&d)[96], uint64_t da, uint64_t db, uint32_t scale_d) {
  asm volatile(
      "{\n\t.reg .pred p;\n\tsetp.ne.b32 p, %98, 0;\n\t"
      "wgmma.mma_async.sync.aligned.m64n192k16.f32.f16.f16 {%0, %1, %2, %3, %4, %5, %6, %7, %8, %9, %10, %11, %12, %13, %14, %15, %16, %17, %18, %19, %20, %21, %22, %23, %24, %25, %26, %27, %28, %29, %30, %31, %32, %33, %34, %35, %36, %37, %38, %39, %40, %41, %42, %43, %44, %45, %46, %47, %48, %49, %50, %51, %52, %53, %54, %55, %56, %57, %58, %59, %60, %61, %62, %63, %64, %65, %66, %67, %68, %69, %70, %71, %72, %73, %74, %75, %76, %77, %78, %79, %80, %81, %82, %83, %84, %85, %86, %87, %88, %89, %90, %91, %92, %93, %94, %95}, %96, %97, p, 1, 1, 0, 0;\n\t}\n"
      : "+f"(d[0]), "+f"(d[1]), "+f"(d[2]), "+f"(d[3]), "+f"(d[4]), "+f"(d[5]), "+f"(d[6]), "+f"(d[7]), "+f"(d[8]), "+f"(d[9]), "+f"(d[10]), "+f"(d[11]), "+f"(d[12]), "+f"(d[13]), "+f"(d[14]), "+f"(d[15]), "+f"(d[16]), "+f"(d[17]), "+f"(d[18]), "+f"(d[19]), "+f"(d[20]), "+f"(d[21]), "+f"(d[22]), "+f"(d[23]), "+f"(d[24]), "+f"(d[25]), "+f"(d[26]), "+f"(d[27]), "+f"(d[28]), "+f"(d[29]), "+f"(d[30]), "+f"(d[31]), "+f"(d[32]), "+f"(d[33]), "+f"(d[34]), "+f"(d[35]), "+f"(d[36]), "+f"(d[37]), "+f"(d[38]), "+f"(d[39]), "+f"(d[40]), "+f"(d[41]), "+f"(d[42]), "+f"(d[43]), "+f"(d[44]), "+f"(d[45]), "+f"(d[46]), "+f"(d[47]), "+f"(d[48]), "+f"(d[49]), "+f"(d[50]), "+f"(d[51]), "+f"(d[52]), "+f"(d[53]), "+f"(d[54]), "+f"(d[55]), "+f"(d[56]), "+f"(d[57]), "+f"(d[58]), "+f"(d[59]), "+f"(d[60]), "+f"(d[61]), "+f"(d[62]), "+f"(d[63]), "+f"(d[64]), "+f"(d[65]), "+f"(d[66]), "+f"(d[67]), "+f"(d[68]), "+f"(d[69]), "+f"(d[70]), "+f"(d[71]), "+f"(d[72]), "+f"(d[73]), "+f"(d[74]), "+f"(d[75]), "+f"(d[76]), "+f"(d[77]), "+f"(d[78]), "+f"(d[79]), "+f"(d[80]), "+f"(d[81]), "+f"(d[82]), "+f"(d[83]), "+f"(d[84]), "+f"(d[85]), "+f"(d[86]), "+f"(d[87]), "+f"(d[88]), "+f"(d[89]), "+f"(d[90]), "+f"(d[91]), "+f"(d[92]), "+f"(d[93]), "+f"(d[94]), "+f"(d[95])
      : "l"(da), "l"(db), "r"(scale_d));
}
__device__ __forceinline__ void wgmma_ss_n256(float (&d)[128], uint64_t da, uint64_t db, uint32_t scale_d) {
  asm volatile(
      "{\n\t.reg .pred p;\n\tsetp.ne.b32 p, %130, 0;\n\t"
      "wgmma.mma_async.sync.aligned.m64n256k16.f32.f16.f16 {%0, %1, %2, %3, %4, %5, %6, %7, %8, %9, %10, %11, %12, %13, %14, %15, %16, %17, %18, %19, %20, %21, %22, %23, %24, %25, %26, %27, %28, %29, %30, %31, %32, %33, %34, %35, %36, %37, %38, %39, %40, %41, %42, %43, %44, %45, %46, %47, %48, %49, %50, %51, %52, %53, %54, %55, %56, %57, %58, %59, %60, %61, %62, %63, %64, %65, %66, %67, %68, %69, %70, %71, %72, %73, %74, %75, %76, %77, %78, %79, %80, %81, %82, %83, %84, %85, %86, %87, %88, %89, %90, %91, %92, %93, %94, %95, %96, %97, %98, %99, %100, %101, %102, %103, %104, %105, %106, %107, %108, %109, %110, %111, %112, %113, %114, %115, %116, %117, %118, %119, %120, %121, %122, %123, %124, %125, %126, %127}, %128, %129, p, 1, 1, 0, 0;\n\t}\n"
      : "+f"(d[0]), "+f"(d[1]), "+f"(d[2]), "+f"(d[3]), "+f"(d[4]), "+f"(d[5]), "+f"(d[6]), "+f"(d[7]), "+f"(d[8]), "+f"(d[9]), "+f"(d[10]), "+f"(d[11]), "+f"(d[12]), "+f"(d[13]), "+f"(d[14]), "+f"(d[15]), "+f"(d[16]), "+f"(d[17]), "+f"(d[18]), "+f"(d[19]), "+f"(d[20]), "+f"(d[21]), "+f"(d[22]), "+f"(d[23]), "+f"(d[24]), "+f"(d[25]), "+f"(d[26]), "+f"(d[27]), "+f"(d[28]), "+f"(d[29]), "+f"(d[30]), "+f"(d[31]), "+f"(d[32]), "+f"(d[33]), "+f"(d[34]), "+f"(d[35]), "+f"(d[36]), "+f"(d[37]), "+f"(d[38]), "+f"(d[39]), "+f"(d[40]), "+f"(d[41]), "+f"(d[42]), "+f"(d[43]), "+f"(d[44]), "+f"(d[45]), "+f"(d[46]), "+f"(d[47]), "+f"(d[48]), "+f"(d[49]), "+f"(d[50]), "+f"(d[51]), "+f"(d[52]), "+f"(d[53]), "+f"(d[54]), "+f"(d[55]), "+f"(d[56]), "+f"(d[57]), "+f"(d[58]), "+f"(d[59]), "+f"(d[60]), "+f"(d[61]), "+f"(d[62]), "+f"(d[63]), "+f"(d[64]), "+f"(d[65]), "+f"(d[66]), "+f"(d[67]), "+f"(d[68]), "+f"(d[69]), "+f"(d[70]), "+f"(d[71]), "+f"(d[72]), "+f"(d[73]), "+f"(d[74]), "+f"(d[75]), "+f"(d[76]), "+f"(d[77]), "+f"(d[78]), "+f"(d[79]), "+f"(d[80]), "+f"(d[81]), "+f"(d[82]), "+f"(d[83]), "+f"(d[84]), "+f"(d[85]), "+f"(d[86]), "+f"(d[87]), "+f"(d[88]), "+f"(d[89]), "+f"(d[90]), "+f"(d[91]), "+f"(d[92]), "+f"(d[93]), "+f"(d[94]), "+f"(d[95]), "+f"(d[96]), "+f"(d[97]), "+f"(d[98]), "+f"(d[99]), "+f"(d[100]), "+f"(d[101]), "+f"(d[102]), "+f"(d[103]), "+f"(d[104]), "+f"(d[105]), "+f"(d[106]), "+f"(d[107]), "+f"(d[108]), "+f"(d[109]), "+f"(d[110]), "+f"(d[111]), "+f"(d[112]), "+f"(d[113]), "+f"(d[114]), "+f"(d[115]), "+f"(d[116]), "+f"(d[117]), "+f"(d[118]), "+f"(d[119]), "+f"(d[120]), "+f"(d[121]), "+f"(d[122]), "+f"(d[123]), "+f"(d[124]), "+f"(d[125]), "+f"(d[126]), "+f"(d[127])
      : "l"(da), "l"(db), "r"(scale_d));
}
__device__ __forceinline__ void wgmma_rs_n64_tb(float (&d)[32], const uint32_t (&a)[4], uint64_t db, uint32_t scale_d) {
  asm volatile(
      "{\n\t.reg .pred p;\n\tsetp.ne.b32 p, %37, 0;\n\t"
      "wgmma.mma_async.sync.aligned.m64n64k16.f32.f16.f16 {%0, %1, %2, %3, %4, %5, %6, %7, %8, %9, %10, %11, %12, %13, %14, %15, %16, %17, %18, %19, %20, %21, %22, %23, %24, %25, %26, %27, %28, %29, %30, %31}, {%32, %33, %34, %35}, %36, p, 1, 1, 1;\n\t}\n"
      : "+f"(d[0]), "+f"(d[1]), "+f"(d[2]), "+f"(d[3]), "+f"(d[4]), "+f"(d[5]), "+f"(d[6]), "+f"(d[7]), "+f"(d[8]), "+f"(d[9]), "+f"(d[10]), "+f"(d[11]), "+f"(d[12]), "+f"(d[13]), "+f"(d[14]), "+f"(d[15]), "+f"(d[16]), "+f"(d[17]), "+f"(d[18]), "+f"(d[19]), "+f"(d[20]), "+f"(d[21]), "+f"(d[22]), "+f"(d[23]), "+f"(d[24]), "+f"(d[25]), "+f"(d[26]), "+f"(d[27]), "+f"(d[28]), "+f"(d[29]), "+f"(d[30]), "+f"(d[31])
      : "r"(a[0]), "r"(a[1]), "r"(a[2]), "r"(a[3]), "l"(db), "r"(scale_d));
}

template <int N> struct WgmmaSS;
template <> struct WgmmaSS<32> { static __device__ __forceinline__ void run(float (&d)[16], uint64_t a, uint64_t b, uint32_t s) { wgmma_ss_n32(d, a, b, s); } };
template <> struct WgmmaSS<64> { static __device__ __forceinline__ void run(float (&d)[32], uint64_t a, uint64_t b, uint32_t s) { wgmma_ss_n64(d, a, b, s); } };
template <> struct WgmmaSS<128> { static __device__ __forceinline__ void run(float (&d)[64], uint64_t a, uint64_t b, uint32_t s) { wgmma_ss_n128(d, a, b, s); } };
template <> struct WgmmaSS<192> { static __device__ __forceinline__ void run(float (&d)[96], uint64_t a, uint64_t b, uint32_t s) { wgmma_ss_n192(d, a, b, s); } };
template <> struct WgmmaSS<256> { static __device__ __forceinline__ void run(float (&d)[128], uint64_t a, uint64_t b, uint32_t s) { wgmma_ss_n256(d, a, b, s); } };

__device__ __forceinline__ uint64_t pack2(float lo, float hi) {
  uint64_t d;
  asm("mov.b64 %0, {%1, %2};" : "=l"(d) : "f"(lo), "f"(hi));
  return d;
}
__device__ __forceinline__ uint64_t pack2u(uint32_t lo, uint32_t hi) {
  uint64_t d;
  asm("mov.b64 %0, {%1, %2};" : "=l"(d) : "r"(lo), "r"(hi));
  return d;
}
__device__ __forceinline__ void unpack2(uint64_t v, float& lo, float& hi) {
  asm("mov.b64 {%0, %1}, %2;" : "=f"(lo), "=f"(hi) : "l"(v));
}
__device__ __forceinline__ uint64_t fma2(uint64_t a, uint64_t b, uint64_t c) {
  float a0, a1, b0, b1, c0, c1;
  unpack2(a, a0, a1);
  unpack2(b, b0, b1);
  unpack2(c, c0, c1);
  return pack2(fmaf(a0, b0, c0), fmaf(a1, b1, c1));
}
__device__ __forceinline__ uint64_t mul2(uint64_t a, uint64_t b) {
  float a0, a1, b0, b1;
  unpack2(a, a0, a1);
  unpack2(b, b0, b1);
  return pack2(__fmul_rn(a0, b0), __fmul_rn(a1, b1));
}

__device__ __forceinline__ float gelu_erf(float x) {
  return 0.5f * x * (1.0f + erff(x * 0.70710678118654752440f));
}
__device__ __forceinline__ float gelu_erf_fast(float x) {
  const float z = fabsf(x) * 0.70710678118654752440f;
  float t;
  asm("rcp.approx.ftz.f32 %0, %1;" : "=f"(t) : "f"(fmaf(0.3275911f, z, 1.0f)));
  float poly = fmaf(t, 1.061405429f, -1.453152027f);
  poly = fmaf(poly, t, 1.421413741f);
  poly = fmaf(poly, t, -0.284496736f);
  poly = fmaf(poly, t, 0.254829592f);
  poly *= t;
  float e;
  asm("ex2.approx.ftz.f32 %0, %1;" : "=f"(e) : "f"(z * z * -1.4426950408889634f));
  const float erf_abs = fmaf(-poly, e, 1.0f);
  const float h = 0.5f * x;
  return fmaf(copysignf(erf_abs, x), h, h);
}
__device__ __forceinline__ void gelu_erf_pair(float& x0, float& x1) {
  const float z0 = fabsf(x0) * 0.70710678118654752440f, z1 = fabsf(x1) * 0.70710678118654752440f;
  const uint64_t z = pack2(z0, z1);
  uint64_t q = fma2(z, pack2(0.0000430638f, 0.0000430638f), pack2(0.0002765672f, 0.0002765672f));
  q = fma2(q, z, pack2(0.0001520143f, 0.0001520143f));
  q = fma2(q, z, pack2(0.0092705272f, 0.0092705272f));
  q = fma2(q, z, pack2(0.0422820123f, 0.0422820123f));
  q = fma2(q, z, pack2(0.0705230784f, 0.0705230784f));
  q = fma2(q, z, pack2(1.0f, 1.0f));
  q = mul2(q, q);
  q = mul2(q, q);
  q = mul2(q, q);
  q = mul2(q, q);
  float p0, p1, r0, r1;
  unpack2(q, p0, p1);
  asm("rcp.approx.ftz.f32 %0, %1;" : "=f"(r0) : "f"(p0));
  asm("rcp.approx.ftz.f32 %0, %1;" : "=f"(r1) : "f"(p1));
  const float h0 = 0.5f * x0, h1 = 0.5f * x1;
  x0 = fmaf(copysignf(1.0f - r0, x0), h0, h0);
  x1 = fmaf(copysignf(1.0f - r1, x1), h1, h1);
}
__device__ __forceinline__ float leaky(float x) { return x > 0.f ? x : 0.01f * x; }

__device__ __forceinline__ uint32_t pack_half2(float a, float b) {
  __half2 h = __floats2half2_rn(a, b);
  return *reinterpret_cast<uint32_t*>(&h);
}

}
```

Before: 213.9.

## Rework GEMM into 2-CTA clusters with multicast B and ping-pong warpgroups

The GEMM kernel now runs as 2-CTA clusters. Each CTA loads its own M tile and half of the B tile, and TMA multicasts that half to both CTAs, which halves weight traffic per CTA. The two consumer warpgroups now alternate whole 128xBN tiles, ordered through named barriers, so one warpgroup's epilogue overlaps the other's MMA. Tile widths are capped at 128 (with a new 96 option) so the doubled accumulator fits in registers, and the stage count is derived from the shared memory left over. This adds cross-CTA barrier arrivals, cluster syncs and smaller N tiles, and the LN partition logic moves into a shared helper exported through the C API.

```diff
diff --git a/include/udb.h b/include/udb.h
--- a/include/udb.h
+++ b/include/udb.h
@@ -61,6 +61,7 @@
 } udb_gemm_t;
 
 int udb_gemm_f16(const udb_gemm_t* g, void* stream);
+int udb_gemm_ln_partition(int32_t N, int32_t* parts, int32_t* part_cols);
 
 typedef struct udb_conv_halo_t {
   const void* x;
diff --git a/unidepth_b200/_cabi.py b/unidepth_b200/_cabi.py
--- a/unidepth_b200/_cabi.py
+++ b/unidepth_b200/_cabi.py
@@ -181,6 +181,7 @@
     "udb_profile_begin": (i32, [vp]),
     "udb_profile_end": (i32, [C.POINTER(ProfileEntry), i32]),
     "udb_gemm_f16": (i32, [C.POINTER(Gemm), vp]),
+    "udb_gemm_ln_partition": (i32, [i32, C.POINTER(i32), C.POINTER(i32)]),
     "udb_conv3x3_halo_f16": (i32, [C.POINTER(ConvHalo), vp]),
     "udb_attention_f16": (i32, [C.POINTER(Attn), vp]),
     "udb_layernorm": (i32, [C.POINTER(LayerNorm), vp]),
diff --git a/unidepth_b200/csrc/engine.cu b/unidepth_b200/csrc/engine.cu
--- a/unidepth_b200/csrc/engine.cu
+++ b/unidepth_b200/csrc/engine.cu
@@ -74,8 +74,8 @@
   const bool sp = e->scalars.count("precision") && e->scalars["precision"] == 1.0;
   const int sx = sp ? 2 : 1;
   const bool fuse = !sp && e->scalars.count("fuse_ln") && e->scalars["fuse_ln"] == 1.0;
-  const int ln_bn = D % 256 == 0 ? 256 : (D % 192 == 0 ? 192 : (D % 128 == 0 ? 128 : 64));
-  const int ln_parts = D / ln_bn * 2, ln_pc = ln_bn / 2;
+  int32_t ln_parts = 0, ln_pc = 0;
+  if (fuse && udb_gemm_ln_partition(D, &ln_parts, &ln_pc)) return 1;
   __half* x16 = fuse ? ar.h(BT * D) : nullptr;
   float* stats = fuse ? ar.f(BT * ln_parts * 2) : nullptr;
   __half* patches = ar.h(BN * 640 * sx);
diff --git a/unidepth_b200/csrc/gemm.cu b/unidepth_b200/csrc/gemm.cu
--- a/unidepth_b200/csrc/gemm.cu
+++ b/unidepth_b200/csrc/gemm.cu
@@ -8,6 +8,8 @@
 constexpr int kEpiWarps = 8;
 constexpr int kTP = 36;
 constexpr int kThreads = (kEpiWarps + 4) * 32;
+constexpr int kCluster = 2;
+constexpr int kOrderBar = 3;
 
 struct GemmArgs {
   int M, N, K, num_kb;
@@ -42,11 +44,12 @@
 
 template <int BN>
 struct GemmCfg {
-  static constexpr int kStages = BN >= 256 ? 3 : (BN >= 192 ? 4 : (BN >= 128 ? 5 : 7));
+  static_assert(BN % 32 == 0 && BN <= 128, "one warpgroup holds the 128 x BN accumulator in at most 128 registers");
   static constexpr int kABytes = BM * BK * 2;
   static constexpr int kBBytes = BN * BK * 2;
   static constexpr int kStageBytes = kABytes + kBBytes;
   static constexpr int kStagingBytes = kEpiWarps * (32 * kTP * 4 + 2 * 32 * 4);
+  static constexpr int kStages = (232448 - kStagingBytes - 256) / kStageBytes;
   static constexpr int kSmemBytes = kStages * kStageBytes + kStagingBytes + 256 ;
   static_assert(kSmemBytes <= 232448, "shared memory per block");
 };
@@ -56,16 +59,13 @@
   float* Twg;
   uint32_t* roff_out;
   uint32_t* roff_res;
-  int wg, wq, grp, lane, r_in_tile;
+  int wg, wq, lane, r_in_tile;
 };
 
 template <int BN, bool LNF>
-__device__ __forceinline__ void epilogue_tile(const GemmArgs& p, const EpiWarp& w, const float (&acc)[BN / 2], const int mt,
+__device__ __forceinline__ void epilogue_tile(const GemmArgs& p, const EpiWarp& w, const float (&acc)[2][BN / 2], const int mt,
                                               const int nt) {
-  constexpr int kGroups = BN >= 64 ? 2 : 1;
-  constexpr int kColsPerGrp = BN / kGroups;
-  const int grp = w.grp, lane = w.lane, r_in_tile = w.r_in_tile;
-  const bool active = grp < kGroups;
+  const int lane = w.lane, r_in_tile = w.r_in_tile;
   float* T = w.T;
   uint32_t* roff_out = w.roff_out;
   uint32_t* roff_res = w.roff_res;
@@ -75,70 +75,65 @@
   float ln_mean = 0.f, ln_rstd = 1.f;
   float st_pivot = 0.f, st_s1 = 0.f, st_s2 = 0.f;
   bool st_first = true;
-  if (active) {
-
-    const int m = mt * BM + r_in_tile;
-    if (p.store_mode == UDB_STORE_CONVTILE || p.store_mode == UDB_STORE_HEAD) {
-      const int per_img = p.conv_tx * p.conv_ty;
-      const int b = mt / per_img;
-      const int r = mt % per_img;
-      const int y = (r / p.conv_tx) * p.conv_TH + r_in_tile / p.conv_TW;
-      const int x = (r % p.conv_tx) * p.conv_TW + r_in_tile % p.conv_TW;
-      valid = (b < p.conv_B) && (y < p.conv_H) && (x < p.conv_W);
-      out_off = (((long long)b * p.conv_H + y) * p.conv_W + x) * p.ldc;
-      res_off = (((long long)b * p.conv_H + y) * p.conv_W + x) * p.ldr;
-    } else if (p.store_mode == UDB_STORE_CONVT) {
-      valid = m < p.M;
-      const int hw = p.ct_h * p.ct_w;
-      const int b = m / hw;
-      const int r = m % hw;
-      const int y = r / p.ct_w, x = r % p.ct_w;
-      const long long W2 = (long long)p.ct_w * p.ct_k + 2 * p.ct_pad;
-      const long long H2 = (long long)p.ct_h * p.ct_k + 2 * p.ct_pad;
-      out_off = ((b * H2 + (long long)y * p.ct_k + p.ct_pad) * W2 + (long long)x * p.ct_k + p.ct_pad) * p.ct_cout;
-      res_off = out_off;
-    } else {
-      valid = m < p.M;
-      long long orow = m;
-      if (p.rpg > 0) orow = (long long)(m / p.rpg) * p.gstride + (m % p.rpg) + p.roff;
-      out_off = orow * p.ldc;
-      res_off = (p.resid_mod > 0) ? ((long long)(m % p.resid_mod) + p.resid_roff) * p.ldr
-                                  : orow * p.ldr;
-    }
-    vmask = __ballot_sync(0xffffffffu, valid);
-    roff_out[lane] = static_cast<uint32_t>(out_off);
-    roff_res[lane] = static_cast<uint32_t>(res_off);
-    __syncwarp();
-    if (LNF && p.ln_stats) {
-      const float2* sp = reinterpret_cast<const float2*>(p.ln_stats) + (long long)(valid ? m : 0) * p.ln_parts;
-      float ms = 0.f, m2 = 0.f;
-      for (int q = 0; q < p.ln_parts; ++q) ms += sp[q].x;
-      ln_mean = ms / (float)p.ln_parts;
-      for (int q = 0; q < p.ln_parts; ++q) {
-        const float2 t = sp[q];
-        m2 += t.y + (float)p.ln_part_cols * (t.x - ln_mean) * (t.x - ln_mean);
-      }
-      ln_rstd = rsqrtf(m2 / (float)(p.ln_parts * p.ln_part_cols) + p.ln_eps);
-    }
+  const int m = mt * BM + r_in_tile;
+  if (p.store_mode == UDB_STORE_CONVTILE || p.store_mode == UDB_STORE_HEAD) {
+    const int per_img = p.conv_tx * p.conv_ty;
+    const int b = mt / per_img;
+    const int r = mt % per_img;
+    const int y = (r / p.conv_tx) * p.conv_TH + r_in_tile / p.conv_TW;
+    const int x = (r % p.conv_tx) * p.conv_TW + r_in_tile % p.conv_TW;
+    valid = (b < p.conv_B) && (y < p.conv_H) && (x < p.conv_W);
+    out_off = (((long long)b * p.conv_H + y) * p.conv_W + x) * p.ldc;
+    res_off = (((long long)b * p.conv_H + y) * p.conv_W + x) * p.ldr;
+  } else if (p.store_mode == UDB_STORE_CONVT) {
+    valid = m < p.M;
+    const int hw = p.ct_h * p.ct_w;
+    const int b = m / hw;
+    const int r = m % hw;
+    const int y = r / p.ct_w, x = r % p.ct_w;
+    const long long W2 = (long long)p.ct_w * p.ct_k + 2 * p.ct_pad;
+    const long long H2 = (long long)p.ct_h * p.ct_k + 2 * p.ct_pad;
+    out_off = ((b * H2 + (long long)y * p.ct_k + p.ct_pad) * W2 + (long long)x * p.ct_k + p.ct_pad) * p.ct_cout;
+    res_off = out_off;
+  } else {
+    valid = m < p.M;
+    long long orow = m;
+    if (p.rpg > 0) orow = (long long)(m / p.rpg) * p.gstride + (m % p.rpg) + p.roff;
+    out_off = orow * p.ldc;
+    res_off = (p.resid_mod > 0) ? ((long long)(m % p.resid_mod) + p.resid_roff) * p.ldr
+                                : orow * p.ldr;
+  }
+  vmask = __ballot_sync(0xffffffffu, valid);
+  roff_out[lane] = static_cast<uint32_t>(out_off);
+  roff_res[lane] = static_cast<uint32_t>(res_off);
+  __syncwarp();
+  if (LNF && p.ln_stats) {
+    const float2* sp = reinterpret_cast<const float2*>(p.ln_stats) + (long long)(valid ? m : 0) * p.ln_parts;
+    float ms = 0.f, m2 = 0.f;
+    for (int q = 0; q < p.ln_parts; ++q) ms += sp[q].x;
+    ln_mean = ms / (float)p.ln_parts;
+    for (int q = 0; q < p.ln_parts; ++q) {
+      const float2 t = sp[q];
+      m2 += t.y + (float)p.ln_part_cols * (t.x - ln_mean) * (t.x - ln_mean);
+    }
+    ln_rstd = rsqrtf(m2 / (float)(p.ln_parts * p.ln_part_cols) + p.ln_eps);
   }
   const int frow = 16 * (w.wq & 1) + (lane >> 2), fcol = 2 * (lane & 3);
 #pragma unroll
-  for (int c = 0; c < kColsPerGrp; c += 32) {
+  for (int c = 0; c < BN; c += 32) {
     bar_sync(1 + w.wg, 128);
 #pragma unroll
-    for (int gi = 0; gi < kGroups; ++gi) {
-      float* Tt = w.Twg + ((w.wq >> 1) | (gi << 1)) * 32 * kTP;
+    for (int h = 0; h < 2; ++h) {
+      float* Tt = w.Twg + ((w.wq >> 1) | (h << 1)) * 32 * kTP;
 #pragma unroll
       for (int j = 0; j < 4; ++j) {
-        const int f = ((gi * kColsPerGrp + c) / 8 + j) * 4;
-        *reinterpret_cast<float2*>(Tt + frow * kTP + 8 * j + fcol) = make_float2(acc[f], acc[f + 1]);
-        *reinterpret_cast<float2*>(Tt + (frow + 8) * kTP + 8 * j + fcol) = make_float2(acc[f + 2], acc[f + 3]);
+        const int f = (c / 8 + j) * 4;
+        *reinterpret_cast<float2*>(Tt + frow * kTP + 8 * j + fcol) = make_float2(acc[h][f], acc[h][f + 1]);
+        *reinterpret_cast<float2*>(Tt + (frow + 8) * kTP + 8 * j + fcol) = make_float2(acc[h][f + 2], acc[h][f + 3]);
       }
     }
     bar_sync(1 + w.wg, 128);
-    if (!active) continue;
-    const int col = grp * kColsPerGrp + c;
-    const int n0 = nt * BN + col;
+    const int n0 = nt * BN + c;
     float v[32];
 #pragma unroll
     for (int j = 0; j < 32; j += 4) {
@@ -303,12 +298,12 @@
       __syncwarp();
     }
   }
-  if (LNF && p.stats_out && active && valid && !st_first) {
-    const float n = (float)kColsPerGrp;
+  if (LNF && p.stats_out && valid && !st_first) {
+    const float n = (float)BN;
     const float mean_p = st_pivot + st_s1 / n;
     const float m2_p = fmaxf(st_s2 - st_s1 * st_s1 / n, 0.f);
     const long long orow = out_off / p.ldc;
-    reinterpret_cast<float2*>(p.stats_out)[orow * (p.tiles_n * kGroups) + nt * kGroups + grp] = make_float2(mean_p, m2_p);
+    reinterpret_cast<float2*>(p.stats_out)[orow * p.tiles_n + nt] = make_float2(mean_p, m2_p);
   }
 }
 
@@ -336,51 +331,55 @@
     prefetch_tmap(&tmB);
     for (int i = 0; i < kStages; ++i) {
       mbar_init(&full_bar[i], 1);
-      mbar_init(&empty_bar[i], kEpiWarps);
+      mbar_init(&empty_bar[i], kCluster * kEpiWarps / 2);
     }
     fence_barrier_init();
   }
-  __syncthreads();
+  cluster_sync();
   pdl_wait();
 
-  const int num_tiles = p.tiles_m * p.tiles_n;
+  const uint32_t rank = cluster_ctarank();
+  const int num_pairs = (p.tiles_m + 1) / 2 * p.tiles_n;
+  const int first_pair = blockIdx.x / kCluster, num_clusters = gridDim.x / kCluster;
 
   if (warp >= kEpiWarps) {
     setmaxnreg_dec<40>();
-    if (warp != kEpiWarps) return;
-    const bool elected = elect_one();
-    int stage = 0;
-    uint32_t phase = 0;
-    for (int tile = blockIdx.x; tile < num_tiles; tile += gridDim.x) {
-      const int mt = tile / p.tiles_n;
-      const int nt = tile % p.tiles_n;
-      int cb = 0, cy = 0, cx = 0;
-      if (p.a_mode == UDB_A_CONV3X3) {
-        const int per_img = p.conv_tx * p.conv_ty;
-        cb = mt / per_img;
-        const int r = mt % per_img;
-        cy = (r / p.conv_tx) * p.conv_TH + p.conv_off;
-        cx = (r % p.conv_tx) * p.conv_TW + p.conv_off;
-      }
-      for (int kb = 0; kb < p.num_kb; ++kb) {
-        mbar_wait(&empty_bar[stage], phase ^ 1);
-        if (elected) {
-          mbar_arrive_expect_tx(&full_bar[stage], Cfg::kStageBytes);
-          if (p.a_mode == UDB_A_CONV3X3) {
-            const int tap = kb / p.conv_cpb;
-            const int c0 = p.conv_coff + (kb % p.conv_cpb) * BK;
-            tma_load_4d(sA + stage * Cfg::kABytes, &tmA, &full_bar[stage], c0, cx + tap % 3, cy + tap / 3, cb);
-          } else {
-            int ka = kb * BK;
-            if (p.a_wrap && ka >= p.a_wrap) ka -= p.a_wrap;
-            tma_load_2d(sA + stage * Cfg::kABytes, &tmA, &full_bar[stage], ka, mt * BM);
+    if (warp == kEpiWarps) {
+      const bool elected = elect_one();
+      int stage = 0;
+      uint32_t phase = 0;
+      for (int pair = first_pair; pair < num_pairs; pair += num_clusters) {
+        const int mt = min(2 * (pair / p.tiles_n) + (int)rank, p.tiles_m - 1);
+        const int nt = pair % p.tiles_n;
+        int cb = 0, cy = 0, cx = 0;
+        if (p.a_mode == UDB_A_CONV3X3) {
+          const int per_img = p.conv_tx * p.conv_ty;
+          cb = mt / per_img;
+          const int r = mt % per_img;
+          cy = (r / p.conv_tx) * p.conv_TH + p.conv_off;
+          cx = (r % p.conv_tx) * p.conv_TW + p.conv_off;
+        }
+        for (int kb = 0; kb < p.num_kb; ++kb) {
+          mbar_wait(&empty_bar[stage], phase ^ 1);
+          if (elected) {
+            mbar_arrive_expect_tx(&full_bar[stage], Cfg::kStageBytes);
+            if (p.a_mode == UDB_A_CONV3X3) {
+              const int tap = kb / p.conv_cpb;
+              const int c0 = p.conv_coff + (kb % p.conv_cpb) * BK;
+              tma_load_4d(sA + stage * Cfg::kABytes, &tmA, &full_bar[stage], c0, cx + tap % 3, cy + tap / 3, cb);
+            } else {
+              int ka = kb * BK;
+              if (p.a_wrap && ka >= p.a_wrap) ka -= p.a_wrap;
+              tma_load_2d(sA + stage * Cfg::kABytes, &tmA, &full_bar[stage], ka, mt * BM);
+            }
+            tma_load_2d_multicast(sB + stage * Cfg::kBBytes + rank * (Cfg::kBBytes / 2), &tmB, &full_bar[stage], kb * BK,
+                                  nt * BN + rank * (BN / 2), (1u << kCluster) - 1);
           }
-          tma_load_2d(sB + stage * Cfg::kBBytes, &tmB, &full_bar[stage], kb * BK, nt * BN);
-        }
-        __syncwarp();
-        if (++stage == kStages) {
-          stage = 0;
-          phase ^= 1;
+          __syncwarp();
+          if (++stage == kStages) {
+            stage = 0;
+            phase ^= 1;
+          }
         }
       }
     }
@@ -389,44 +388,67 @@
     const int wg = warp >> 2, wq = warp & 3;
     float* Twg = reinterpret_cast<float*>(staging) + wg * 4 * 32 * kTP;
     uint32_t* roff = reinterpret_cast<uint32_t*>(staging + kEpiWarps * 32 * kTP * 4) + warp * 64;
-    const EpiWarp ctx{Twg + wq * 32 * kTP, Twg, roff, roff + 32, wg, wq, wq >> 1, lane, 64 * wg + 32 * (wq & 1) + lane};
-    float acc[BN / 2];
-#pragma unroll
-    for (int i = 0; i < BN / 2; ++i) acc[i] = 0.f;
+    const EpiWarp ctx{Twg + wq * 32 * kTP, Twg, roff, roff + 32, wg, wq, lane, 32 * wq + lane};
+    float acc[2][BN / 2];
+#pragma unroll
+    for (int i = 0; i < BN / 2; ++i) acc[0][i] = acc[1][i] = 0.f;
     int stage = 0;
     uint32_t phase = 0;
-    for (int tile = blockIdx.x; tile < num_tiles; tile += gridDim.x) {
-      const int mt = tile / p.tiles_n;
-      const int nt = tile % p.tiles_n;
+    auto skip_tile = [&]() {
+      stage += p.num_kb;
+      phase ^= (stage / kStages) & 1;
+      stage %= kStages;
+    };
+    if (wg == 1) skip_tile();
+    auto release = [&](int s) {
+      if (lane == 0)
+        for (uint32_t c = 0; c < kCluster; ++c) mbar_arrive_cluster(&empty_bar[s], c);
+    };
+    for (int pair = first_pair + wg * num_clusters, i = wg; pair < num_pairs; pair += 2 * num_clusters, i += 2) {
+      const int mt = 2 * (pair / p.tiles_n) + (int)rank;
+      const int nt = pair % p.tiles_n;
+      if (i > 0) bar_sync(kOrderBar + wg, 256);
       int prev = -1;
       for (int kb = 0; kb < p.num_kb; ++kb) {
         mbar_wait(&full_bar[stage], phase);
-        const uint64_t da = gmma_desc_sw128(smem_u32(sA + stage * Cfg::kABytes + wg * 64 * 128), 16, 1024);
+        const uint64_t da0 = gmma_desc_sw128(smem_u32(sA + stage * Cfg::kABytes), 16, 1024);
+        const uint64_t da1 = gmma_desc_sw128(smem_u32(sA + stage * Cfg::kABytes + 64 * 128), 16, 1024);
         const uint64_t db = gmma_desc_sw128(smem_u32(sB + stage * Cfg::kBBytes), 16, 1024);
         wgmma_fence();
 #pragma unroll
-        for (int k = 0; k < BK / 16; ++k) WgmmaSS<BN>::run(acc, da + 2 * k, db + 2 * k, (kb | k) != 0 ? 1u : 0u);
+        for (int k = 0; k < BK / 16; ++k) {
+          WgmmaSS<BN>::run(acc[0], da0 + 2 * k, db + 2 * k, (kb | k) != 0 ? 1u : 0u);
+          WgmmaSS<BN>::run(acc[1], da1 + 2 * k, db + 2 * k, (kb | k) != 0 ? 1u : 0u);
+        }
         wgmma_commit();
         wgmma_wait<1>();
-        if (prev >= 0 && lane == 0) mbar_arrive(&empty_bar[prev]);
+        if (prev >= 0) release(prev);
         prev = stage;
         if (++stage == kStages) {
           stage = 0;
           phase ^= 1;
         }
       }
+      if (pair + num_clusters < num_pairs) bar_arrive(kOrderBar + (wg ^ 1), 256);
       wgmma_wait<0>();
-      wgmma_fence_regs(acc);
-      if (prev >= 0 && lane == 0) mbar_arrive(&empty_bar[prev]);
+      wgmma_fence_regs(acc[0]);
+      wgmma_fence_regs(acc[1]);
+      if (prev >= 0) release(prev);
       epilogue_tile<BN, LNF>(p, ctx, acc, mt, nt);
-    }
-  }
+      skip_tile();
+    }
+  }
+  cluster_sync();
 }
 
 template <int BN, bool LNF>
 static int launch_gemm(const CUtensorMap& tmA, const CUtensorMap& tmB, const GemmArgs& a, cudaStream_t st) {
   using Cfg = GemmCfg<BN>;
   static std::atomic<uint64_t> attr_mask{0};
+  static int max_clusters[64];
+  int dev = 0;
+  cudaGetDevice(&dev);
+  if (dev >= 64) { set_error("gemm: device ordinal %d", dev); return 1; }
   if (first_on_device(attr_mask)) {
     cudaError_t e = cudaFuncSetAttribute(gemm_f16_kernel<BN, LNF>, cudaFuncAttributeMaxDynamicSharedMemorySize,
                                          Cfg::kSmemBytes);
@@ -434,10 +456,29 @@
       set_error("gemm: cudaFuncSetAttribute(%d B smem): %s", Cfg::kSmemBytes, cudaGetErrorString(e));
       return 1;
     }
-  }
-  const int tiles = a.tiles_m * a.tiles_n;
-  const int grid = tiles < num_sms() ? tiles : num_sms();
-  cudaError_t e = launch_ex(gemm_f16_kernel<BN, LNF>, dim3(grid), dim3(kThreads), Cfg::kSmemBytes, st, 1, tmA, tmB, a);
+    cudaLaunchConfig_t cfg{};
+    cfg.gridDim = dim3(kCluster * num_sms());
+    cfg.blockDim = dim3(kThreads);
+    cfg.dynamicSmemBytes = Cfg::kSmemBytes;
+    cudaLaunchAttribute attr;
+    attr.id = cudaLaunchAttributeClusterDimension;
+    attr.val.clusterDim.x = kCluster;
+    attr.val.clusterDim.y = 1;
+    attr.val.clusterDim.z = 1;
+    cfg.attrs = &attr;
+    cfg.numAttrs = 1;
+    int n = 0;
+    e = cudaOccupancyMaxActiveClusters(&n, gemm_f16_kernel<BN, LNF>, &cfg);
+    if (e != cudaSuccess || n <= 0) {
+      set_error("gemm: cudaOccupancyMaxActiveClusters: %s (%d)", cudaGetErrorString(e), n);
+      return 1;
+    }
+    max_clusters[dev] = n;
+  }
+  const int pairs = (a.tiles_m + 1) / 2 * a.tiles_n;
+  const int clusters = pairs < max_clusters[dev] ? pairs : max_clusters[dev];
+  cudaError_t e = launch_ex(gemm_f16_kernel<BN, LNF>, dim3(kCluster * clusters), dim3(kThreads), Cfg::kSmemBytes, st,
+                            kCluster, tmA, tmB, a);
   if (e != cudaSuccess) {
     set_error("gemm_f16_kernel launch: %s", cudaGetErrorString(e));
     return 1;
@@ -445,6 +486,26 @@
   return check_launch("gemm_f16_kernel");
 }
 
+static int ln_partition(int N, int* parts, int* part_cols) {
+  const int w = N % 256 == 0 ? 256 : (N % 192 == 0 ? 192 : (N % 128 == 0 ? 128 : (N % 64 == 0 ? 64 : 0)));
+  if (N <= 0 || w == 0) {
+    set_error("udb_gemm_ln_partition: N=%d must be a positive multiple of 64", N);
+    return 1;
+  }
+  *part_cols = w / 2;
+  *parts = N / *part_cols;
+  return 0;
+}
+
+}
+
+extern "C" int udb_gemm_ln_partition(int32_t N, int32_t* parts, int32_t* part_cols) {
+  if (!parts || !part_cols) { udb::set_error("udb_gemm_ln_partition: null output"); return 1; }
+  int p = 0, c = 0;
+  if (udb::ln_partition(N, &p, &c)) return 1;
+  *parts = p;
+  *part_cols = c;
+  return 0;
 }
 
 extern "C" int udb_gemm_f16(const udb_gemm_t* g, void* stream) {
@@ -490,23 +551,22 @@
   if (g->store_mode == UDB_STORE_HEAD) {
     if (g->N != 32) { set_error("udb_gemm_f16: HEAD store needs N == 32"); return 1; }
     bn = 32;
-  } else if (g->N % 256 == 0) bn = 256;
-  else if (g->N % 192 == 0) bn = 192;
-  else if (g->N % 128 == 0) bn = 128;
+  } else if (g->ln_stats_out) {
+    int parts = 0;
+    if (ln_partition(g->N, &parts, &bn)) return 1;
+    if (g->ln_parts != parts || g->ln_part_cols != bn) {
+      set_error("udb_gemm_f16: ln_stats_out with N=%d runs as %d parts of %d columns (caller said %d x %d)", g->N, parts, bn,
+                g->ln_parts, g->ln_part_cols);
+      return 1;
+    }
+  } else if (g->N % 128 == 0) bn = 128;
+  else if (g->N % 96 == 0) bn = 96;
   else if (g->N % 64 == 0) bn = 64;
   else bn = 32;
   if (g->store_mode == UDB_STORE_CONVT && (g->ct_cout % 32) != 0) {
     set_error("udb_gemm_f16: CONVT needs Cout %% 32 == 0"); return 1;
   }
   a.tiles_n = (g->N + bn - 1) / bn;
-  if (g->ln_stats_out) {
-    const int groups = bn >= 64 ? 2 : 1;
-    if (g->N % bn || g->ln_parts != a.tiles_n * groups || g->ln_part_cols != bn / groups) {
-      set_error("udb_gemm_f16: ln_stats_out with N=%d runs as %d parts of %d columns (caller said %d x %d)", g->N, a.tiles_n * groups,
-                bn / groups, g->ln_parts, g->ln_part_cols);
-      return 1;
-    }
-  }
 
   CUtensorMap tmA, tmB;
   if (g->a_mode == UDB_A_CONV3X3) {
@@ -546,7 +606,7 @@
   {
     const uint64_t dims[2] = {(uint64_t)g->K, (uint64_t)g->N};
     const uint64_t str[1] = {(uint64_t)g->ldw * 2};
-    const uint32_t box[2] = {(uint32_t)BK, (uint32_t)bn};
+    const uint32_t box[2] = {(uint32_t)BK, (uint32_t)(bn / kCluster)};
     if (make_tmap_f16(&tmB, g->w, 2, dims, str, box, true)) return 1;
   }
   cudaStream_t st = reinterpret_cast<cudaStream_t>(stream);
@@ -556,17 +616,15 @@
   const bool lnf = g->ln_stats_out || g->ln_stats_in;
   if (lnf) {
     switch (bn) {
-      case 256: return launch_gemm<256, true>(tmA, tmB, a, st);
-      case 192: return launch_gemm<192, true>(tmA, tmB, a, st);
       case 128: return launch_gemm<128, true>(tmA, tmB, a, st);
+      case 96: return launch_gemm<96, true>(tmA, tmB, a, st);
       case 64: return launch_gemm<64, true>(tmA, tmB, a, st);
       default: return launch_gemm<32, true>(tmA, tmB, a, st);
     }
   }
   switch (bn) {
-    case 256: return launch_gemm<256, false>(tmA, tmB, a, st);
-    case 192: return launch_gemm<192, false>(tmA, tmB, a, st);
     case 128: return launch_gemm<128, false>(tmA, tmB, a, st);
+    case 96: return launch_gemm<96, false>(tmA, tmB, a, st);
     case 64: return launch_gemm<64, false>(tmA, tmB, a, st);
     default: return launch_gemm<32, false>(tmA, tmB, a, st);
   }
diff --git a/unidepth_b200/csrc/ptx.cuh b/unidepth_b200/csrc/ptx.cuh
--- a/unidepth_b200/csrc/ptx.cuh
+++ b/unidepth_b200/csrc/ptx.cuh
@@ -42,6 +42,23 @@
                "r"(bytes)
                : "memory");
 }
+__device__ __forceinline__ void mbar_arrive_cluster(uint64_t* bar, uint32_t cta) {
+  asm volatile(
+      "{\n\t.reg .b32 ra;\n\t"
+      "mapa.shared::cluster.u32 ra, %0, %1;\n\t"
+      "mbarrier.arrive.shared::cluster.b64 _, [ra];\n\t}\n" ::"r"(smem_u32(bar)),
+      "r"(cta)
+      : "memory");
+}
+__device__ __forceinline__ uint32_t cluster_ctarank() {
+  uint32_t r;
+  asm volatile("mov.u32 %0, %%cluster_ctarank;" : "=r"(r));
+  return r;
+}
+__device__ __forceinline__ void cluster_sync() {
+  asm volatile("barrier.cluster.arrive.release.aligned;\n\tbarrier.cluster.wait.acquire.aligned;" ::: "memory");
+}
+
 __device__ __forceinline__ bool mbar_try_wait(uint64_t* bar, uint32_t parity) {
   uint32_t ok;
   asm volatile(
@@ -81,6 +98,14 @@
       "l"(reinterpret_cast<uint64_t>(tmap)), "r"(smem_u32(bar)), "r"(c0), "r"(c1)
       : "memory");
 }
+__device__ __forceinline__ void tma_load_2d_multicast(void* smem_dst, const void* tmap, uint64_t* bar, int c0, int c1,
+                                                      uint16_t cta_mask) {
+  asm volatile(
+      "cp.async.bulk.tensor.2d.shared::cluster.global.mbarrier::complete_tx::bytes.multicast::cluster"
+      " [%0], [%1, {%3, %4}], [%2], %5;" ::"r"(smem_u32(smem_dst)),
+      "l"(reinterpret_cast<uint64_t>(tmap)), "r"(smem_u32(bar)), "r"(c0), "r"(c1), "h"(cta_mask)
+      : "memory");
+}
 __device__ __forceinline__ void tma_load_3d(void* smem_dst, const void* tmap, uint64_t* bar, int c0,
                                             int c1, int c2) {
   asm volatile(
@@ -116,6 +141,9 @@
 __device__ __forceinline__ void setmaxnreg_dec() { asm volatile("setmaxnreg.dec.sync.aligned.u32 %0;" ::"n"(R)); }
 __device__ __forceinline__ void bar_sync(int id, int threads) {
   asm volatile("bar.sync %0, %1;" ::"r"(id), "r"(threads) : "memory");
+}
+__device__ __forceinline__ void bar_arrive(int id, int threads) {
+  asm volatile("bar.arrive %0, %1;" ::"r"(id), "r"(threads) : "memory");
 }
 
 __device__ __forceinline__ uint64_t gmma_desc_sw128(uint32_t smem_addr, uint32_t lbo_bytes, uint32_t sbo_bytes) {
@@ -141,6 +169,13 @@
       : "+f"(d[0]), "+f"(d[1]), "+f"(d[2]), "+f"(d[3]), "+f"(d[4]), "+f"(d[5]), "+f"(d[6]), "+f"(d[7]), "+f"(d[8]), "+f"(d[9]), "+f"(d[10]), "+f"(d[11]), "+f"(d[12]), "+f"(d[13]), "+f"(d[14]), "+f"(d[15]), "+f"(d[16]), "+f"(d[17]), "+f"(d[18]), "+f"(d[19]), "+f"(d[20]), "+f"(d[21]), "+f"(d[22]), "+f"(d[23]), "+f"(d[24]), "+f"(d[25]), "+f"(d[26]), "+f"(d[27]), "+f"(d[28]), "+f"(d[29]), "+f"(d[30]), "+f"(d[31])
       : "l"(da), "l"(db), "r"(scale_d));
 }
+__device__ __forceinline__ void wgmma_ss_n96(float (&d)[48], uint64_t da, uint64_t db, uint32_t scale_d) {
+  asm volatile(
+      "{\n\t.reg .pred p;\n\tsetp.ne.b32 p, %50, 0;\n\t"
+      "wgmma.mma_async.sync.aligned.m64n96k16.f32.f16.f16 {%0, %1, %2, %3, %4, %5, %6, %7, %8, %9, %10, %11, %12, %13, %14, %15, %16, %17, %18, %19, %20, %21, %22, %23, %24, %25, %26, %27, %28, %29, %30, %31, %32, %33, %34, %35, %36, %37, %38, %39, %40, %41, %42, %43, %44, %45, %46, %47}, %48, %49, p, 1, 1, 0, 0;\n\t}\n"
+      : "+f"(d[0]), "+f"(d[1]), "+f"(d[2]), "+f"(d[3]), "+f"(d[4]), "+f"(d[5]), "+f"(d[6]), "+f"(d[7]), "+f"(d[8]), "+f"(d[9]), "+f"(d[10]), "+f"(d[11]), "+f"(d[12]), "+f"(d[13]), "+f"(d[14]), "+f"(d[15]), "+f"(d[16]), "+f"(d[17]), "+f"(d[18]), "+f"(d[19]), "+f"(d[20]), "+f"(d[21]), "+f"(d[22]), "+f"(d[23]), "+f"(d[24]), "+f"(d[25]), "+f"(d[26]), "+f"(d[27]), "+f"(d[28]), "+f"(d[29]), "+f"(d[30]), "+f"(d[31]), "+f"(d[32]), "+f"(d[33]), "+f"(d[34]), "+f"(d[35]), "+f"(d[36]), "+f"(d[37]), "+f"(d[38]), "+f"(d[39]), "+f"(d[40]), "+f"(d[41]), "+f"(d[42]), "+f"(d[43]), "+f"(d[44]), "+f"(d[45]), "+f"(d[46]), "+f"(d[47])
+      : "l"(da), "l"(db), "r"(scale_d));
+}
 __device__ __forceinline__ void wgmma_ss_n128(float (&d)[64], uint64_t da, uint64_t db, uint32_t scale_d) {
   asm volatile(
       "{\n\t.reg .pred p;\n\tsetp.ne.b32 p, %66, 0;\n\t"
@@ -173,6 +208,7 @@
 template <int N> struct WgmmaSS;
 template <> struct WgmmaSS<32> { static __device__ __forceinline__ void run(float (&d)[16], uint64_t a, uint64_t b, uint32_t s) { wgmma_ss_n32(d, a, b, s); } };
 template <> struct WgmmaSS<64> { static __device__ __forceinline__ void run(float (&d)[32], uint64_t a, uint64_t b, uint32_t s) { wgmma_ss_n64(d, a, b, s); } };
+template <> struct WgmmaSS<96> { static __device__ __forceinline__ void run(float (&d)[48], uint64_t a, uint64_t b, uint32_t s) { wgmma_ss_n96(d, a, b, s); } };
 template <> struct WgmmaSS<128> { static __device__ __forceinline__ void run(float (&d)[64], uint64_t a, uint64_t b, uint32_t s) { wgmma_ss_n128(d, a, b, s); } };
 template <> struct WgmmaSS<192> { static __device__ __forceinline__ void run(float (&d)[96], uint64_t a, uint64_t b, uint32_t s) { wgmma_ss_n192(d, a, b, s); } };
 template <> struct WgmmaSS<256> { static __device__ __forceinline__ void run(float (&d)[128], uint64_t a, uint64_t b, uint32_t s) { wgmma_ss_n256(d, a, b, s); } };
```

Measured after the change: 222.4 (median of 6 runs). 4.0% higher.
